# amoretti86/phylo

Measured on AMD Instinct MI355X. Metric: particle-site-likelihoods/sec, higher is better.
Workload: dtype f64; 1 GPU; primate.p N=12 S=898, GTR-init (jcmodel=false), K=2048 per GPU (K_total=2048), lambda=10, full sweep of 11 rank events; parallelism=particles sharded over 1 GPU(s), global resampling, sweeps_per_launch_set=16, contexts_in_flight=3, sweeps_in_flight=48, particles_in_flight=98304

## Files before the change

### phylo_amd/csrc/phylo_hip.hip

```cpp
#include "../../include/phylo_hip.h"

#include <cstring>
#include <hip/hip_runtime.h>
#include <hip/hip_ext.h>
#include <rocprim/device/device_radix_sort.hpp>

#include <cstdarg>
#include <cstdio>
#include <cstdlib>
#include <atomic>
#include <chrono>
#include <mutex>
#include <string>
#include <vector>

#include "phylo_comm.h"
#include "phylo_kernels.h"
#include "phylo_packed_codes.h"
#include "phylo_site_patterns.h"
#include "phylo_persist.h"
#include "phylo_grad.h"
#include "phylo_revlists_dev.h"
#include "phylo_sweep_plan.h"
#include "phylo_train.h"
// ... 27 lines not shown
    uint64_t seed = 0;
    uint32_t flags = 0;
    int M = 1, launches = 0, next_r = 0;
    bool active = false;
    int a_done_r = -1;
    sweep_plan plan{};
    sweep_chain_form chain{};
};

struct env_switches {
    bool eager_nodes = false, rehearse_sharded = false, replicated_book = false, no_leaf_codes = false, one_launch = false,
         persist_stamps = false, grad_one_stream = false, grad_two_streams = false, rev_host_lists = false, no_remote_cache = false,
         no_p2p = false, grad_rows_chain = false, grad_coeff_chain = false, tree_wide_keys = false;
    int persist_wgs = 0;
    unsigned long long p2p_wait_ticks = PK_P2P_WAIT_TICKS;
    size_t p2p_copy_words = 65536;
    int persist_nt = 256;
    int remote_cache_cap = 0;
    int scan_multi_min = 4096;
    int scan_ancestors = 1;
    int site_patterns = PK_PAT_AUTO;
    int clade_patterns = PK_CLADE_AUTO;
    int trees_chunk = 0;
    int launch_xcd = 0;
    int rell_chunk = 0;
    void read() {
        eager_nodes = getenv("PHYLO_EAGER_NODES") != nullptr;
        rehearse_sharded = getenv("PHYLO_REHEARSE_SHARDED") != nullptr;
        replicated_book = getenv("PHYLO_REPLICATED_BOOK") != nullptr;
        grad_rows_chain = getenv("PHYLO_GRAD_ROWS_CHAIN") != nullptr;
        grad_coeff_chain = getenv("PHYLO_GRAD_COEFF_CHAIN") != nullptr;
        no_leaf_codes = getenv("PHYLO_NO_LEAF_CODES") != nullptr;
        one_launch = getenv("PHYLO_ONE_LAUNCH") != nullptr;
        persist_stamps = getenv("PHYLO_PERSIST_STAMPS") != nullptr;
        grad_one_stream = getenv("PHYLO_GRAD_ONE_STREAM") != nullptr;
        grad_two_streams = getenv("PHYLO_GRAD_TWO_STREAMS") != nullptr;
        rev_host_lists = getenv("PHYLO_REV_HOST_LISTS") != nullptr;
        no_remote_cache = getenv("PHYLO_NO_REMOTE_CACHE") != nullptr;
        { const char* e = getenv("PHYLO_TREE_WIDE_KEYS"); tree_wide_keys = e && atoi(e) != 0; }
        { const char* e = getenv("PHYLO_REMOTE_CACHE_CAP"); remote_cache_cap = e ? atoi(e) : 0; }
        { const char* e = getenv("PHYLO_SITE_PATTERNS"); site_patterns = !e ? PK_PAT_AUTO : !strcmp(e, "force") ? PK_PAT_FORCE : atoi(e) == 0 ? PK_PAT_OFF : PK_PAT_AUTO; }
        { const char* e = getenv("PHYLO_CLADE_PATTERNS"); clade_patterns = !e ? PK_CLADE_AUTO : !strcmp(e, "force") ? PK_CLADE_FORCE : atoi(e) == 0 ? PK_CLADE_OFF : PK_CLADE_AUTO; }
        { const char* e = getenv("PHYLO_SCAN_MULTI_MIN"); scan_multi_min = e ? atoi(e) : 4096; }
        { const char* e = getenv("PHYLO_SCAN_ANCESTORS"); scan_ancestors = e ? atoi(e) : 1; }
        { const char* e = getenv("PHYLO_TREES_CHUNK"); trees_chunk = e ? atoi(e) : 0; }
        { const char* e = getenv("PHYLO_RELL_CHUNK"); rell_chunk = e ? atoi(e) : 0; }
        { const char* e = getenv("PHYLO_LAUNCH_XCD"); launch_xcd = !e ? 0 : atoi(e) > 0 ? atoi(e) : -1; }
        { const char* e = getenv("PHYLO_P2P"); no_p2p = e && atoi(e) == 0; }
        { const char* e = getenv("PHYLO_P2P_COPY_WORDS"); p2p_copy_words = e ? (size_t)atol(e) : 65536; }
        { const char* e = getenv("PHYLO_P2P_WAIT_S"); p2p_wait_ticks = e && atof(e) > 0 ? (unsigned long long)(atof(e) * 1e8) : PK_P2P_WAIT_TICKS; }
        const char* w = getenv("PHYLO_PERSIST_WGS");
        persist_wgs = w ? atoi(w) : 0;
        const char* t = getenv("PHYLO_PERSIST_NT");
        persist_nt = persist_nt_of(t ? atoi(t) : 0);
    }
};

struct phylo_ctx {
    int device = 0;
    env_switches env;
    int n_cus = 0;
    unsigned long long* d_rdraw = nullptr;
    unsigned long long* d_pctr = nullptr;
    unsigned long long pctr_base = 0;
    int pctr_Wg = 0, pctr_G = 0;
    bool pctr_dirty = false;
    int persist_blocks_per_cu = -1;
    bool last_persistent = false;
    int last_pp_nt = 0, last_pp_Wg = 0, last_pp_m = 0;
    size_t last_pp_lds = 0;
    unsigned long long* d_stamps = nullptr;
    int K = 0, N = 0, S = 0, A = 4;
    int Kloc = 0, k0 = 0;
    int rank = 0, world = 1;
    uint32_t flags = 0;
    hipStream_t stream = nullptr;
    hipEvent_t ev0 = nullptr, ev1 = nullptr;
    std::vector<hipEvent_t> kev;
    std::string err;
    bool have_leaves = false, have_model = false, swept = false, state_ready = false;
    int jc = 0;
    std::vector<double> h_lam_l, h_lam_r, h_ldf;
    double *d_Q = nullptr, *d_pi = nullptr, *d_lam_l = nullptr, *d_lam_r = nullptr, *d_ldf = nullptr;
    double* d_leaves = nullptr;
    uint8_t* d_leaf_codes = nullptr;
    uint8_t* d_leaf_packed = nullptr;
    uint8_t* d_pat = nullptr;
    int pat_U = 0;
    bool leaves_coded = false;
    uint8_t* d_clade = nullptr;
    uint8_t* h_clade_p = nullptr;
    size_t clade_cap = 0;
    pk_clade_layout clade_layout{};
    bool clade_ready = false;
    hipEvent_t ev_clade = nullptr;
    int32_t* d_bits[2] = {nullptr, nullptr};
    uint32_t* d_pair_hist = nullptr;
    bool hist_ready = false, codes_valid = false;
    double* d_pool = nullptr;
    double* d_nodell = nullptr;
    double *d_bl = nullptr, *d_br = nullptr, *d_Pmat = nullptr;
    double *d_logw = nullptr, *d_ll = nullptr;
    double* d_aux = nullptr;
    unsigned long long* d_rec = nullptr;
    int tile_override = 0;
    int site_tile = 0, ntiles = 1;
    double* d_tilev = nullptr;
    double* d_lse = nullptr;
    uint64_t* d_group_seeds = nullptr;
    char* d_tables = nullptr;
    int32_t *d_roots[2] = {nullptr, nullptr}, *d_cnt[2] = {nullptr, nullptr};
    double* d_rootll[2] = {nullptr, nullptr};
    const char** d_tab_ptrs = nullptr;
    int32_t* d_child = nullptr;
    unsigned int* d_mark = nullptr;
    double* d_sync = nullptr;
    bool p2p = false;
    char* d_xslab = nullptr;
    size_t xslab_bytes = 0, x_flag_off[2] = {0, 0};
    char** d_xslab_ptrs = nullptr;
    unsigned long long x_epoch[2] = {0, 0};
    bool last_lazy = false;
    bool leaves_newer = false;
    int32_t* d_merges = nullptr;
    int64_t* d_anc = nullptr;
    uint64_t* d_cdf[2] = {nullptr, nullptr};
    int32_t* d_anc_next = nullptr;
    int32_t* d_adopt_list = nullptr;
    int32_t* d_adopt_cnt = nullptr;
    int last_chain = 0;
    unsigned int* d_counter = nullptr;
    const double** d_pool_ptrs = nullptr;
    int32_t* d_mirror = nullptr;
    double* d_cache = nullptr;
    int cache_cap = 0;
    int32_t *d_roots_ad = nullptr, *d_cnt_ad = nullptr;
    double *d_rootll_ad = nullptr, *d_chosen = nullptr, *d_tw_b = nullptr, *d_tw_P = nullptr, *d_pot = nullptr;
    size_t tw_capacity = 0;
    double* d_twbuf = nullptr;
    size_t twbuf_cap = 0;
    double *d_htw_b = nullptr, *d_htw_P = nullptr, *d_hpot = nullptr, *d_hchosen = nullptr;
    int32_t* d_hroots_ad = nullptr;
    double *d_tau = nullptr, *d_ctw = nullptr, *d_twpart = nullptr, *d_twnode = nullptr;
    int64_t* d_joff = nullptr;
    size_t htw_rows = 0;
    std::vector<int64_t> h_joff;
    bool last_graph_twist = false, last_graph_marks = false;
    bool last_graph_eager = false;
    int last_M = 1;
    int32_t *d_hroots = nullptr, *d_hcnt = nullptr, *d_pos = nullptr;
    double* d_hrootll = nullptr;
    double *d_adj = nullptr, *d_om = nullptr, *d_G = nullptr, *d_C = nullptr, *d_part = nullptr, *d_nodeg = nullptr;
    double *d_leafpi = nullptr, *d_leafterm = nullptr, *d_terms = nullptr, *d_gout = nullptr;
    int32_t *d_ad_off = nullptr, *d_ad_idx = nullptr, *d_par_off = nullptr, *d_par_idx = nullptr;
    int32_t *d_heavy = nullptr, *d_chunk_beg = nullptr, *d_chunk_cnt = nullptr;
    int32_t *d_slow_flag = nullptr, *d_slow_idx = nullptr, *d_adp = nullptr;
    bool graph_ready = false, last_graph = false;
    int last_G = 1;
    bool last_final_missing = false;
    std::vector<uint64_t> h_group_seeds;
    int64_t* h_anc_p = nullptr;
    std::vector<int64_t> h_anc_glob;
    std::vector<double> h_gout;
    double* h_model_p = nullptr;
    double* h_leaves_p = nullptr;
    hipEvent_t ev_leaves = nullptr;
// ... 344 lines not shown
        HIPCHK(c, hipHostGetDevicePointer((void**)&c->hd_csr, c->h_csr_p, 0));
        HIPCHK(c, hipHostGetDevicePointer((void**)&c->hd_anc, c->h_anc_p, 0));
        HIPCHK(c, hipHostGetDevicePointer((void**)&c->hd_child, c->h_child_p, 0));
        HIPCHK(c, hipHostMalloc((void**)&c->h_pub, 16));
        HIPCHK(c, hipHostGetDevicePointer((void**)&c->hd_pub, c->h_pub, 0));
        HIPCHK(c, hipEventCreateWithFlags(&c->ev_gcopy, hipEventDisableTiming));
        HIPCHK(c, hipHostMalloc((void**)&c->h_dlmeta, ((size_t)PG_DL_META_INTS(R) + 4) * 4));
        c->h_dlmeta[PG_DL_META_INTS(R)] = 0;
        HIPCHK(c, hipHostGetDevicePointer((void**)&c->hd_dlmeta, c->h_dlmeta, 0));
        HIPCHK(c, hipEventCreateWithFlags(&c->ev_dl, hipEventDisableTiming));
        c->dl_temp_nn = 0;
        const pg_lists D = pg_lists_carve(c->d_ad_off, R, K);
        c->d_ad_idx = D.ad_idx; c->d_par_off = D.par_off; c->d_par_idx = D.par_idx;
        c->d_heavy = D.heavy; c->d_chunk_beg = D.chunk_beg; c->d_chunk_cnt = D.chunk_cnt;
        c->d_slow_flag = D.slow_flag; c->d_slow_idx = D.slow_idx; c->d_adp = D.adp;
    }
    if (c->world > 1) {
        const size_t Kl = c->Kloc, W = c->world;
        CHK(dalloc(c, &c->d_gchild, R * K * 2));
        CHK(dalloc(c, &c->d_gbl, R * K));
        CHK(dalloc(c, &c->d_gbr, R * K));
        CHK(dalloc(c, &c->d_gPmat, R * K * 32));
        CHK(dalloc(c, &c->d_ganc, (R > 1 ? R - 1 : 1) * K));
        c->gx_seg = R * Kl * 36 + (R > 1 ? (R - 1) * Kl : 0);
        c->gx_cl = c->gx_seg < PHYLO_SHM_SLOT / 8 ? c->gx_seg : PHYLO_SHM_SLOT / 8;
        const size_t words = (c->gx_seg + c->gx_cl - 1) / c->gx_cl * c->gx_cl * W;
        void* buf = nullptr;
        if (hipExtMallocWithFlags(&buf, words * 8, hipDeviceMallocFinegrained) != hipSuccess) {
            (void)hipGetLastError();
            HIPCHK(c, hipMalloc(&buf, words * 8));
        }
        c->d_gx = (unsigned long long*)buf;
        CHK(dalloc(c, &c->d_gx_src, W));
        std::vector<void*> src(W, buf);
        if (c->p2p) {
            int rc = phylo_comm_map_extra(c->comm, buf, &src, c->stream, &c->err);
            if (rc != PHYLO_OK) return rc;
        }
        HIPCHK(c, hipMemcpy((void*)c->d_gx_src, src.data(), W * sizeof(void*), hipMemcpyHostToDevice));
    }
    if (!c->evb0) {
        HIPCHK(c, hipEventCreate(&c->evb0));
        HIPCHK(c, hipEventCreate(&c->evb1));
        HIPCHK(c, hipStreamCreateWithFlags(&c->gstream, hipStreamNonBlocking));
        HIPCHK(c, hipEventCreateWithFlags(&c->ev_gfork, hipEventDisableTiming));
        HIPCHK(c, hipEventCreateWithFlags(&c->ev_gjoin, hipEventDisableTiming));
        HIPCHK(c, hipEventCreateWithFlags(&c->ev_gup, hipEventDisableTiming));
        {
            int least = 0, greatest = 0;
            HIPCHK(c, hipDeviceGetStreamPriorityRange(&least, &greatest));
            HIPCHK(c, hipStreamCreateWithPriority(&c->bgstream, hipStreamNonBlocking, least));
        }
        HIPCHK(c, hipEventCreateWithFlags(&c->ev_bgfork, hipEventDisableTiming));
        HIPCHK(c, hipEventCreateWithFlags(&c->ev_bgdone, hipEventDisableTiming));
        c->ev_coeff.assign((size_t)R, nullptr);
        for (auto& e : c->ev_coeff) HIPCHK(c, hipEventCreateWithFlags(&e, hipEventDisableTiming));
    }
    c->graph_ready = true;
    return PHYLO_OK;
}

template <typename... P, typename... A>
void launch_stamped(void (*kernel)(P...), dim3 grid, dim3 block, size_t lds, hipStream_t s, hipEvent_t e0, hipEvent_t e1, A&&... args) {
    if (e0) hipExtLaunchKernelGGL(kernel, grid, block, lds, s, e0, e1, 0, args...);
    else hipLaunchKernelGGL(kernel, grid, block, lds, s, args...);
}

static sweep_limits sweep_limits_of() {
    sweep_limits L{};
    L.max_groups = PK_MAX_GROUPS; L.twist_max_m = PK_TWIST_MAX_M; L.twist_max_j = PK_TWIST_MAX_J;
    L.mat_group = PK_MAT_GROUP; L.scan_fold_max_kg = PP_SCAN_KERNEL_MAX_KG; L.kept_bits_taxa = PG_KEPT_BITS_TAXA;
    L.scan_lds512_max_kg = 4096;
    L.one_tile_max_s = 4096;
    L.small_max_kg = 4096; L.small_max_kloc = 8192;
    L.book_packed8_min = 8192;
    L.sorted_min_draws = 262144;
    return L;
}
static const sweep_limits k_sweep_limits = sweep_limits_of();

int launch_scan(phylo_ctx* c, const double* logw, int Kg, int G, uint64_t* cdf, double* lse, int lse_stride, int logz_R = 0,
                const pp_anc_out* anc = nullptr) {
    const pp_anc_out ao = anc ? *anc : pp_anc_out{};
    const sweep_scan_form form = sweep_scan_form_of(Kg, c->env.scan_multi_min, cdf || lse, k_sweep_limits);
    if (ao.anc && (!cdf || logz_R > 0 || (form != SCAN_LDS_512 && form != SCAN_LDS_1024)))
        return fail(c, PHYLO_ESTATE, "launch_scan: the resampling outcome needs a cdf and a scan that holds it in LDS (Kg = %d)", Kg);
    if (form == SCAN_MULTI) {
        pp_scan_multi_args a{};
        a.logw = logw; a.Kg = Kg; a.B = (Kg + PP_SCAN_TILE - 1) / PP_SCAN_TILE;
        void* ws = nullptr;
        const size_t nb = (size_t)G * a.B;
        CHK(scratch_get(c, 11, (nb * 2 + (size_t)G * Kg) * 8, &ws));
        a.gmax = (double*)ws; a.bsum = (unsigned long long*)ws + nb; a.wbits = (unsigned long long*)ws + 2 * nb;
        a.cdf = (unsigned long long*)cdf; a.lse_out = lse; a.lse_stride = lse_stride; a.logz_R = logz_R;
        hipLaunchKernelGGL(pp_scan_multi_max, dim3(a.B, G), dim3(512), 0, c->stream, a);
        CHK(launch_check(c, "pp_scan_multi_max"));
        hipLaunchKernelGGL(pp_scan_multi_exp, dim3(a.B, G), dim3(512), 0, c->stream, a);
        CHK(launch_check(c, "pp_scan_multi_exp"));
        if (cdf) hipLaunchKernelGGL(pp_scan_multi_cdf, dim3(a.B + 1, G), dim3(512), 0, c->stream, a);
        else { a.lse_only = 1; hipLaunchKernelGGL(pp_scan_multi_cdf, dim3(1, G), dim3(512), 0, c->stream, a); }
        return launch_check(c, "pp_scan_multi_cdf");
    }
    if (form == SCAN_LDS_512) {
        if (ao.anc) hipLaunchKernelGGL(pp_resample_scan_anc<512>, dim3(G), dim3(512), pp_resample_scan_lds(Kg, true), c->stream, logw, Kg, cdf, lse, lse_stride, ao);
        else hipLaunchKernelGGL(pp_resample_scan<512>, dim3(G), dim3(512), pp_resample_scan_lds(Kg), c->stream, logw, Kg, cdf, lse, lse_stride, logz_R);
        return launch_check(c, "pp_resample_scan");
    }
    if (form == SCAN_LDS_1024) {
        const size_t lds = pp_resample_scan_lds(Kg, ao.anc != nullptr);
        static bool raised = false, raised_anc = false;
        if (lds > 65536 && !raised && !ao.anc) {
            HIPCHK(c, hipFuncSetAttribute((const void*)pp_resample_scan<1024>, hipFuncAttributeMaxDynamicSharedMemorySize,
                                          (int)pp_resample_scan_lds(PP_SCAN_KERNEL_MAX_KG)));
            raised = true;
        }
        if (ao.anc) {
            if (lds > 65536 && !raised_anc) {
                HIPCHK(c, hipFuncSetAttribute((const void*)pp_resample_scan_anc<1024>, hipFuncAttributeMaxDynamicSharedMemorySize,
                                              (int)pp_resample_scan_lds(PP_SCAN_KERNEL_MAX_KG, true)));
                raised_anc = true;
            }
            hipLaunchKernelGGL(pp_resample_scan_anc<1024>, dim3(G), dim3(1024), lds, c->stream, logw, Kg, cdf, lse, lse_stride, ao);
            return launch_check(c, "pp_resample_scan_anc");
        }
        hipLaunchKernelGGL(pp_resample_scan<1024>, dim3(G), dim3(1024), lds, c->stream, logw, Kg, cdf, lse, lse_stride, logz_R);
        return launch_check(c, "pp_resample_scan");
    }
    if (G > 1) hipLaunchKernelGGL(pk_resample_scan_groups, dim3(G), dim3(PK_COLS), 0, c->stream, logw, Kg, cdf, lse, lse_stride);
    else hipLaunchKernelGGL(pk_resample_scan, dim3(1), dim3(PK_COLS), 0, c->stream, logw, Kg, cdf, lse);
    return launch_check(c, "pk_resample_scan");
}

int wait_event_spin(phylo_ctx* c, hipEvent_t ev) {
    const auto t0 = std::chrono::steady_clock::now();
    for (;;) {
        const hipError_t e = hipEventQuery(ev);
        if (e == hipSuccess) return PHYLO_OK;
        if (e != hipErrorNotReady) return fail(c, PHYLO_EHIP, "hipEventQuery: %s", hipGetErrorString(e));
        if (std::chrono::steady_clock::now() - t0 > std::chrono::milliseconds(2)) break;
        __builtin_ia32_pause();
    }
    HIPCHK(c, hipEventSynchronize(ev));
    return PHYLO_OK;
}

int tile_for(const phylo_ctx* c, int S) { return c->tile_override ? c->tile_override : pm_site_tile(S); }

int refresh_leaf_ll(phylo_ctx* c) {
    if (!(c->have_leaves && c->have_model && c->state_ready)) return PHYLO_OK;
    hipLaunchKernelGGL(pk_row_loglik, dim3(c->N), dim3(64), 0, c->stream, c->d_leaves, c->d_pi, c->S, c->site_tile,
                       c->d_nodell);
    return launch_check(c, "pk_row_loglik(leaves)");
}

}

extern "C" {

const char* phylo_version(void) { return "phylo_hip 0.1 (gfx950)"; }

const char* phylo_last_error(const phylo_ctx* ctx) { return ctx ? ctx->err.c_str() : g_last_error.c_str(); }

int phylo_device_count(void) {
    int n = 0;
    if (hipGetDeviceCount(&n) != hipSuccess) return 0;
    return n;
}

int phylo_create(const int* device_ids, int n_gpus, int K, int N, int S, int A, uint32_t flags,
                 phylo_ctx** out) {
    if (!out) return fail(nullptr, PHYLO_EINVAL, "out is NULL");
    *out = nullptr;
    if (n_gpus != 1)
        return fail(nullptr, PHYLO_EINVAL, "n_gpus must be 1 (one process per GPU; join ranks with phylo_comm_init)");
    if (A != 4) return fail(nullptr, PHYLO_EINVAL, "A must be 4 (DNA alphabet), got %d", A);
    if (K < 1 || N < 2 || S < 1) return fail(nullptr, PHYLO_EINVAL, "need K >= 1, N >= 2, S >= 1 (K=%d N=%d S=%d)", K, N, S);
    if (N > PK_MAX_TAXA) return fail(nullptr, PHYLO_EINVAL, "N = %d exceeds the supported maximum %d", N, PK_MAX_TAXA);
    if ((double)(N - 1) * K + N > 2.0e9) return fail(nullptr, PHYLO_EINVAL, "node ids overflow int32");
    int ndev = 0;
    hipError_t e = hipGetDeviceCount(&ndev);
    if (e != hipSuccess || ndev < 1)
        return fail(nullptr, PHYLO_ENODEVICE, "no HIP device available (%s); this library has no CPU path",
                    e != hipSuccess ? hipGetErrorString(e) : "device count 0");
    const int dev = device_ids ? device_ids[0] : 0;
    if (dev < 0 || dev >= ndev) return fail(nullptr, PHYLO_ENODEVICE, "device id %d out of range [0,%d)", dev, ndev);
    phylo_ctx* c = new phylo_ctx();
    c->device = dev;
    c->K = K; c->N = N; c->S = S; c->A = A;
    c->Kloc = K; c->k0 = 0;
    c->flags = flags;
    c->env.read();
    {
        const char* t = getenv("PHYLO_SITE_TILE");
        int T = t ? atoi(t) : pm_site_tile(S);
        if (T < 64 || (T & 63) || T > PK_MAX_SITE_TILE) { delete c; return fail(nullptr, PHYLO_EINVAL, "PHYLO_SITE_TILE must be a multiple of 64 in [64, %d] (got %d)", PK_MAX_SITE_TILE, T); }
        c->tile_override = t ? T : 0;
        c->site_tile = T;
        c->ntiles = (S + T - 1) / T;
    }
    int rc = PHYLO_OK;
    do {
        if ((rc = bind(c)) != PHYLO_OK) break;
        {
            hipDeviceProp_t prop;
            if (hipGetDeviceProperties(&prop, dev) != hipSuccess) { rc = fail(c, PHYLO_EHIP, "hipGetDeviceProperties failed"); break; }
            c->n_cus = prop.multiProcessorCount;
        }
        if (hipStreamCreateWithFlags(&c->stream, hipStreamNonBlocking) != hipSuccess) { rc = fail(c, PHYLO_EHIP, "hipStreamCreate failed"); break; }
        if (hipEventCreate(&c->ev0) != hipSuccess || hipEventCreate(&c->ev1) != hipSuccess) { rc = fail(c, PHYLO_EHIP, "hipEventCreate failed"); break; }
        if ((rc = dalloc(c, &c->d_Q, 20 + 2 * (size_t)N)) != PHYLO_OK) break;
        c->d_pi = c->d_Q + 16;
        c->d_lam_l = c->d_Q + 20;
        c->d_lam_r = c->d_Q + 20 + N;
        if ((rc = dalloc(c, &c->d_ldf, (size_t)N + 1)) != PHYLO_OK) break;
        if ((rc = dalloc(c, &c->d_leaves, (size_t)N * S * 4)) != PHYLO_OK) break;
        if ((rc = dalloc(c, &c->d_leaf_codes, pk_leaf_image_bytes(N, S))) != PHYLO_OK) break;
        c->d_leaf_packed = c->d_leaf_codes + pk_packed_offset(N, S);
        c->d_pat = c->d_leaf_codes + pk_pat_offset(N, S);
        c->h_ldf.resize((size_t)N + 1);
        for (int cnt = 0; cnt <= N; ++cnt) c->h_ldf[cnt] = host_log_double_factorial(2 * (cnt > 2 ? cnt : 2) - 3);
        if (hipMemcpy(c->d_ldf, c->h_ldf.data(), ((size_t)N + 1) * 8, hipMemcpyHostToDevice) != hipSuccess) { rc = fail(c, PHYLO_EHIP, "ldf upload failed"); break; }
    } while (0);
    if (rc != PHYLO_OK) {
        g_last_error = c->err;
        phylo_destroy(c);
        return rc;
    }
    *out = c;
    return PHYLO_OK;
}

int phylo_destroy(phylo_ctx* c) {
    if (!c) return PHYLO_OK;
    (void)hipSetDevice(c->device);
    if (c->stream) (void)hipStreamSynchronize(c->stream);
    if (c->gstream) (void)hipStreamSynchronize(c->gstream);
    if (c->bgstream) (void)hipStreamSynchronize(c->bgstream);
    phylo_comm_destroy(&c->comm);
    free_sweep_state(c);
    void* ptrs[] = {c->d_Q, c->d_ldf, c->d_leaves, c->d_leaf_codes, c->d_clade};
    for (void* p : ptrs)
        if (p) (void)hipFree(p);
    for (auto& b : c->scratch)
        if (b.p) (void)hipFree(b.p);
    for (hipEvent_t e : c->kev) (void)hipEventDestroy(e);
    if (c->ev0) (void)hipEventDestroy(c->ev0);
    if (c->ev1) (void)hipEventDestroy(c->ev1);
    if (c->evb0) (void)hipEventDestroy(c->evb0);
    if (c->evb1) (void)hipEventDestroy(c->evb1);
    if (c->ev_model) (void)hipEventDestroy(c->ev_model);
    if (c->ev_tb0) (void)hipEventDestroy(c->ev_tb0);
    if (c->ev_tb1) (void)hipEventDestroy(c->ev_tb1);
    if (c->ev_tl0) (void)hipEventDestroy(c->ev_tl0);
    if (c->ev_tl1) (void)hipEventDestroy(c->ev_tl1);
    if (c->ev_rl0) (void)hipEventDestroy(c->ev_rl0);
    if (c->ev_rl1) (void)hipEventDestroy(c->ev_rl1);
    if (c->ev_rm0) (void)hipEventDestroy(c->ev_rm0);
    if (c->ev_rm1) (void)hipEventDestroy(c->ev_rm1);
    if (c->ev_tg0) (void)hipEventDestroy(c->ev_tg0);
    if (c->ev_tg1) (void)hipEventDestroy(c->ev_tg1);
    if (c->ev_tr0) (void)hipEventDestroy(c->ev_tr0);
    if (c->ev_tr1) (void)hipEventDestroy(c->ev_tr1);
    if (c->ev_tn0) (void)hipEventDestroy(c->ev_tn0);
    if (c->ev_tn1) (void)hipEventDestroy(c->ev_tn1);
    if (c->ev_tm0) (void)hipEventDestroy(c->ev_tm0);
    if (c->ev_tm1) (void)hipEventDestroy(c->ev_tm1);
    if (c->ev_tq0) (void)hipEventDestroy(c->ev_tq0);
    if (c->ev_tq1) (void)hipEventDestroy(c->ev_tq1);
    if (c->ev_ta0) (void)hipEventDestroy(c->ev_ta0);
    if (c->ev_ta1) (void)hipEventDestroy(c->ev_ta1);
    if (c->ev_ts0) (void)hipEventDestroy(c->ev_ts0);
    if (c->ev_ts1) (void)hipEventDestroy(c->ev_ts1);
    if (c->ev_gfork) (void)hipEventDestroy(c->ev_gfork);
    if (c->ev_gjoin) (void)hipEventDestroy(c->ev_gjoin);
    if (c->ev_gup) (void)hipEventDestroy(c->ev_gup);
    if (c->ev_bgfork) (void)hipEventDestroy(c->ev_bgfork);
    if (c->ev_bgdone) (void)hipEventDestroy(c->ev_bgdone);
    if (c->bgstream) (void)hipStreamDestroy(c->bgstream);
    for (hipEvent_t e : c->ev_coeff)
        if (e) (void)hipEventDestroy(e);
    if (c->gstream) (void)hipStreamDestroy(c->gstream);
    if (c->h_model_p) (void)hipHostFree(c->h_model_p);
    if (c->ev_leaves) (void)hipEventDestroy(c->ev_leaves);
    if (c->h_leaves_p) (void)hipHostFree(c->h_leaves_p);
    if (c->ev_clade) (void)hipEventDestroy(c->ev_clade);
    if (c->h_clade_p) (void)hipHostFree(c->h_clade_p);
    if (c->stream) (void)hipStreamDestroy(c->stream);
    delete c;
    return PHYLO_OK;
}

int phylo_site_tile(int S) { return pm_site_tile(S); }

int phylo_get_site_tile(const phylo_ctx* c) { return c ? c->site_tile : 0; }

int phylo_set_site_tile(phylo_ctx* c, int T) {
    CHK(bind(c));
    if (T < 0 || (T & 63) || T > PK_MAX_SITE_TILE)
        return fail(c, PHYLO_EINVAL, "the site tile must be a multiple of 64 in [64, %d], or 0 for the default (got %d)", PK_MAX_SITE_TILE, T);
    if (c->comm.transport != 0) return fail(c, PHYLO_ESTATE, "phylo_set_site_tile must precede phylo_comm_init (peers map the sweep state)");
    HIPCHK(c, hipStreamSynchronize(c->stream));
    c->tile_override = T;
    c->site_tile = T ? T : pm_site_tile(c->S);
    c->ntiles = (c->S + c->site_tile - 1) / c->site_tile;
// ... 1693 lines not shown
    const size_t lds = pp_layout(N, m, Kg).total;
    c->swept = false; ++c->sweep_serial;
    CHK(persist_chain(c, false));
    HIPCHK(c, hipEventRecord(c->ev0, c->stream));
    if (c->env.persist_nt == 512) hipLaunchKernelGGL((pp_sweep<512>), dim3(G * Wg), dim3(512), lds, c->stream, a);
    else hipLaunchKernelGGL((pp_sweep<256>), dim3(G * Wg), dim3(256), lds, c->stream, a);
    CHK(launch_check(c, "pp_sweep"));
    HIPCHK(c, hipEventRecord(c->ev1, c->stream));
    CHK(persist_chain(c, true));
    c->pctr_base += (unsigned long long)R * Wg;
    sweep_publish(c, true, false, G, false, 0, 1, (double)K * S * R);
    c->last_persistent = true;
    c->last_chain = 0;
    c->last_pp_nt = c->env.persist_nt; c->last_pp_Wg = Wg; c->last_pp_m = m; c->last_pp_lds = lds;
    return PHYLO_OK;
}


int phylo_sweep_begin(phylo_ctx* c, uint64_t seed, uint32_t flags, int M) { return sweep_begin_impl(c, seed, flags, M, nullptr, 1); }

static int comm_exchange(phylo_ctx* c, double* const* arrays, int n_arrays, size_t count, int purpose) {
    if (c->comm.transport == 0) return PHYLO_OK;
    if (!c->p2p) {
        if (n_arrays == 0) { double* rows[1] = {c->d_sync}; return phylo_comm_allgather_inplace(c->comm, rows, 1, 1, c->stream, &c->err); }
        return phylo_comm_allgather_inplace(c->comm, arrays, n_arrays, count, c->stream, &c->err);
    }
    if (n_arrays > 4) return fail(c, PHYLO_EINVAL, "comm_exchange: at most four arrays");
    pk_p2p_args a{};
    a.slabs = c->d_xslab_ptrs; a.world = c->world; a.me = c->rank;
    a.n_seg = n_arrays; a.seg_count = (int)count;
    for (int i = 0; i < n_arrays; ++i) {
        const ptrdiff_t off = (const char*)arrays[i] - c->d_xslab;
        if (off < 0 || (size_t)off + (size_t)c->world * count * 8 > c->xslab_bytes) return fail(c, PHYLO_EINVAL, "comm_exchange: array outside the exchange slab");
        a.seg_off[i] = (size_t)off;
    }
    a.flag_off = c->x_flag_off[purpose];
    a.epoch = ++c->x_epoch[purpose];
    a.timeout_word = c->d_counter + 1;
    a.wait_ticks = c->env.p2p_wait_ticks;
    const size_t words = (size_t)n_arrays * count * (size_t)(c->world - 1);
    if (words > c->env.p2p_copy_words) {
        const size_t wgs = (words + 4095) / 4096;
        hipLaunchKernelGGL(pk_p2p_copy, dim3((unsigned)(wgs < 512 ? wgs : 512)), dim3(1024), 0, c->stream, a);
        CHK(launch_check(c, "pk_p2p_copy"));
        a.n_seg = 0;
    }
    hipLaunchKernelGGL(pk_p2p_exchange, dim3(1), dim3(1024), 0, c->stream, a);
    return launch_check(c, "pk_p2p_exchange");
}

static bool pat_on(const phylo_ctx* c) { return pk_pat_take(c->S, c->pat_U, c->leaves_coded, c->ntiles, c->env.site_patterns); }

static pk_rank_args rank_args(const phylo_ctx* c, int r) {
    const sweep_plan& p = c->run.plan;
    const int N = c->N, K = c->K, Kl = c->Kloc, cur = r & 1, nxt = cur ^ 1;
    const size_t plane = (size_t)K * N;
    pk_rank_args b{};
    b.r = r; b.n = N - r; b.N = N; b.S = c->S; b.K = K; b.Kloc = Kl; b.k0 = c->k0;
    b.seed = c->run.seed; b.flags = c->run.flags;
    b.Kg = p.Kg; b.group_seeds = p.G > 1 ? c->d_group_seeds : nullptr;
    b.no_store = (r == p.R - 1 && p.no_store_last) ? 1 : 0;
    if (p.graph) {
        b.roots_old = c->d_hroots + plane * r; b.cnt_old = c->d_hcnt + plane * r;
        b.roots_new = c->d_hroots + plane * (r + 1); b.cnt_new = c->d_hcnt + plane * (r + 1);
        b.rootll_old = c->d_hrootll + plane * r; b.rootll_new = c->d_hrootll + plane * (r + 1);
        b.pos_hist = c->d_pos + plane * r;
    } else {
        b.roots_old = c->d_roots[cur]; b.cnt_old = c->d_cnt[cur];
        b.roots_new = c->d_roots[nxt]; b.cnt_new = c->d_cnt[nxt];
        b.rootll_old = c->d_rootll[cur]; b.rootll_new = c->d_rootll[nxt];
        if (p.clade_pat) { b.bits_old = c->d_bits[cur]; b.bits_new = c->d_bits[nxt]; }
    }
    if (p.local_book) {
        b.tab_ptrs = c->d_tab_ptrs;
        b.tab_off_rootll = (size_t)cur * K * N * 8;
        b.tab_off_roots = (size_t)16 * K * N + (size_t)cur * K * N * 4;
        b.tab_off_cnt = (size_t)24 * K * N + (size_t)cur * K * N * 4;
    }
    b.cdf = c->d_cdf[cur];
    b.rdraw = p.want_rdraw ? c->d_rdraw + (size_t)r * K : nullptr;
    b.ll_prev = r > 0 ? c->d_ll + (size_t)(r - 1) * K : nullptr;
    b.nodell = c->d_nodell;
    b.ldf = c->d_ldf; b.ldf_n = N;
    b.bl = c->d_bl; b.br = c->d_br;
    b.lam_l = c->h_lam_l[r]; b.lam_r = c->h_lam_r[r];
    b.loglam_l = pm_log(b.lam_l); b.loglam_r = pm_log(b.lam_r);
    b.ll_tilde0 = pm_log(1.0 / (double)p.Kg);
    b.leaves = c->d_leaves; b.pool = c->d_pool; b.pool_ptrs = c->d_pool_ptrs;
    b.mirror = (p.twist || p.replicated_book) ? nullptr : c->d_mirror; b.cache = c->d_cache; b.cache_cap = c->cache_cap;
    b.leaf_codes = c->leaves_coded ? c->d_leaf_codes : nullptr;
    b.leaf_packed = c->leaves_coded ? c->d_leaf_packed : nullptr;
    b.packed_leaf_bytes = pk_packed_leaf_bytes(c->S);
    b.Pmat = c->d_Pmat + (size_t)r * Kl * 32;
    b.pi = c->d_pi;
    b.logw_r = c->d_logw + (size_t)r * K;
    b.ll_r = c->d_ll + (size_t)r * K;
    b.merges = c->d_merges; b.ancestors = c->d_anc;
    b.child = c->d_child + (size_t)r * Kl * 2; b.aux = c->d_aux;
    b.rec = p.use_rec ? c->d_rec : nullptr;
    b.lazy = p.lazy ? 1 : 0; b.mark = c->d_mark; b.child_all = c->d_child; b.Pmat_all = c->d_Pmat;
    b.T = c->site_tile; b.ntiles = c->ntiles; b.tilev = c->d_tilev;
    if (c->run.chain.taken && r > 0) {
        b.anc_in = c->d_anc_next; b.adopt_list = c->d_adopt_list; b.adopt_cnt = c->d_adopt_cnt;
        b.item_waves = c->run.chain.item_waves; b.item_parts = c->run.chain.parts;
    }
    b.book_xcd = c->run.chain.taken && p.book_xcd;
    return b;
}

static int step_materialize(phylo_ctx* c, const pk_rank_args& b) {
    const sweep_plan& p = c->run.plan;
    const int Kl = c->Kloc, S = c->S;
    if (c->run.chain.taken) return PHYLO_OK;
    if (p.mat_by_draws) {
        const int grouped = p.mat_draws_grouped ? 1 : 0;
        hipLaunchKernelGGL(pk_materialize_by_draws, dim3(grouped ? Kl / PK_MAT_GROUP : Kl), dim3(PK_COLS), 0, c->stream, b, grouped);
        CHK(launch_check(c, "pk_materialize_by_draws"));
    } else {
        if (p.step_a_work) {
            hipLaunchKernelGGL(pk_all_marks, dim3(cdiv(c->K, 4)), dim3(64), 0, c->stream, b);
            CHK(launch_check(c, "pk_all_marks"));
        }
        if (p.mat_grouped) hipLaunchKernelGGL(pk_materialize_adopted_grouped, dim3(cdiv(Kl, PK_MAT_GROUP)), dim3(PK_COLS), 0, c->stream, b);
        else hipLaunchKernelGGL(pk_materialize_adopted, dim3(p.one_tile ? 1 : cdiv(S, PK_MAT_TILE), Kl), dim3(PK_COLS), 0, c->stream, b);
        CHK(launch_check(c, "pk_materialize_adopted"));
    }
    if (p.mat_barrier) CHK(comm_exchange(c, nullptr, 0, 0, 1));
    return PHYLO_OK;
}

static int sweep_step_a(phylo_ctx* c) {
    CHK(bind(c));
    if (!c->run.active) return fail(c, PHYLO_ESTATE, "phylo_sweep_step without phylo_sweep_begin");
    const int R = c->N - 1, r = c->run.next_r;
    if (r >= R) return fail(c, PHYLO_ESTATE, "all %d rank events of this sweep have been issued", R);
    c->run.a_done_r = r;
    if (!c->run.plan.step_a_work || r == 0) return PHYLO_OK;
    return step_materialize(c, rank_args(c, r));
}

static int step_twist(phylo_ctx* c, const pk_rank_args& b) {
    const sweep_plan& p = c->run.plan;
    const int N = c->N, K = c->K, Kl = c->Kloc, r = b.r;
    pk_twist_args ta{};
    ta.a = b;
    ta.M = c->run.M;
    ta.J = ((N - r) * (N - r - 1) / 2) * ta.M;
    ta.roots_ad = c->d_roots_ad; ta.cnt_ad = c->d_cnt_ad; ta.rootll_ad = c->d_rootll_ad;
    ta.tw_b = c->d_tw_b; ta.tw_P = c->d_tw_P; ta.pot = c->d_pot; ta.chosen = c->d_chosen;
    if (p.graph) {
        const size_t j0 = (size_t)c->h_joff[r];
        ta.tw_b = c->d_htw_b + j0 * 2; ta.tw_P = c->d_htw_P + j0 * 32; ta.pot = c->d_hpot + j0;
        ta.roots_ad = c->d_hroots_ad + (size_t)K * N * r; ta.chosen = c->d_hchosen + (size_t)r * K;
    }
    ta.Pmat_r = c->d_Pmat + (size_t)r * Kl * 32;
    ta.pair_hist = p.twist_ll ? c->d_pair_hist : nullptr;
    ta.codes = p.twist_ll ? c->d_leaf_codes : nullptr;
    ta.bl_r = c->d_bl + (size_t)r * Kl; ta.br_r = c->d_br + (size_t)r * Kl;
    ta.own_tables = p.twist_tables ? 0 : 1;
    ta.wbuf = c->d_twbuf;
    hipLaunchKernelGGL(pk_twist_adopt_draws, dim3(K + cdiv(2L * Kl * ta.J, 64)), dim3(64), 0, c->stream, ta, (const double*)c->d_Q, c->jc);
    CHK(launch_check(c, "pk_twist_adopt_draws"));
    if (p.twist_ll) {
        hipLaunchKernelGGL(pk_twist_potentials_ll, dim3((ta.J + 7) / 8, Kl), dim3(256), 0, c->stream, ta);
        CHK(launch_check(c, "pk_twist_potentials_ll"));
    }
// ... 59 lines not shown
        return launch_check(c, "pk_rank_book_chain");
    }
    const dim3 grid(cdiv(p.local_book ? c->Kloc : K, per));
    if (p.clade_pat) {
        if (w == 8) hipLaunchKernelGGL(pk_rank_book_packed_clade<8>, grid, dim3(64), lds * per, c->stream, b);
        else if (w == 16) hipLaunchKernelGGL(pk_rank_book_packed_clade<16>, grid, dim3(64), lds * per, c->stream, b);
        else return fail(c, PHYLO_ESTATE, "step_book: clade patterns at %d lanes", w);
        return launch_check(c, "pk_rank_book_packed");
    }
    switch (w) {
    case 8: hipLaunchKernelGGL(pk_rank_book_packed<8>, grid, dim3(64), lds * per, c->stream, b); break;
    case 16: hipLaunchKernelGGL(pk_rank_book_packed<16>, grid, dim3(64), lds * per, c->stream, b); break;
    case 32: hipLaunchKernelGGL(pk_rank_book_packed<32>, grid, dim3(64), lds * per, c->stream, b); break;
    case 64: hipLaunchKernelGGL(pk_rank_book_packed<64>, grid, dim3(64), lds * per, c->stream, b); break;
    default: return fail(c, PHYLO_ESTATE, "step_book: no pk_rank_book_packed of %d lanes", w);
    }
    return launch_check(c, "pk_rank_book_packed");
}

static int step_merge(phylo_ctx* c, const pk_rank_args& b) {
    const sweep_plan& p = c->run.plan;
    const int S = c->S;
    const dim3 mgrid((unsigned)((size_t)c->Kloc * c->ntiles));
    hipEvent_t e0 = nullptr, e1 = nullptr;
    if (p.timek && !p.twist) { e0 = c->kev[2 * b.r]; e1 = c->kev[2 * b.r + 1]; }
    if (!(b.lazy || b.no_store)) {
        const size_t lds = (size_t)(c->site_tile < S ? c->site_tile : S) * 8 + 16 + PK_STORE_STAGE_BYTES;
        launch_stamped(pk_rank_merge, mgrid, dim3(PK_COLS), lds, c->stream, e0, e1, b);
    } else if (b.rec) {
        pk_pi4 pi4;
        memcpy(pi4.v, c->h_model_p + 16, sizeof pi4.v);
        pk_pat_args pat = {nullptr, nullptr, 0, 0, 0u, 0u, nullptr};
        size_t lds = 0;
        if (p.clade_pat) {
            const pk_clade_layout& L = c->clade_layout;
            pat.clade = (const char*)c->d_clade + L.codes_bytes;
            pat.cstride = (unsigned int)L.stride; pat.crep = (unsigned int)L.rep_bytes;
            pat.rep_delta = (long long)(c->d_clade - c->d_leaf_packed);
            pat.U = c->pat_U;
            lds = pk_pat_lds_bytes(c->pat_U);
        } else if (pat_on(c)) {
            pat.pimg = (const char*)c->d_pat;
            pat.roff = (const char*)c->d_pat + pk_pat_image_bytes(S);
            pat.rep_delta = (long long)((c->d_pat + pk_pat_image_bytes(S) + pk_pat_rep_bytes()) - c->d_leaf_packed);
            pat.U = c->pat_U;
            lds = pk_pat_lds_bytes(c->pat_U);
        }
        const int n = (int)mgrid.x, grid = pk_launch_grid(n, 1, p.launch_xcd), n_xcd = p.launch_xcd ? -n : n;
        launch_stamped(pk_rank_merge_nostore, dim3((unsigned)grid), dim3(64), lds, c->stream, e0, e1, (const unsigned long long*)b.rec, b.Pmat,
                       S, b.T, b.ntiles, n_xcd, b.tilev, pi4, pat);
    } else {
        launch_stamped(pk_rank_merge_nostore_ids, mgrid, dim3(64), 0, c->stream, e0, e1, b);
    }
    return launch_check(c, "pk_rank_merge");
}

static int step_tiles(phylo_ctx* c, const pk_rank_args& b) {
    hipLaunchKernelGGL(pk_tile_epilogue, dim3(cdiv(c->Kloc, 256)), dim3(256), 0, c->stream, b);
    return launch_check(c, "pk_tile_epilogue");
}

static int step_exchange(phylo_ctx* c, int r) {
    const size_t K = c->K;
    double* rows[3] = {c->d_logw + r * K, c->d_ll + r * K, c->d_nodell + c->N + r * K};
    return comm_exchange(c, rows, 3, (size_t)c->Kloc, 0);
}

static int step_fix_rootll(phylo_ctx* c, int r) {
    const int N = c->N, K = c->K;
    double* rootll_new = c->run.plan.graph ? c->d_hrootll + (size_t)K * N * (r + 1) : c->d_rootll[(r & 1) ^ 1];
    hipLaunchKernelGGL(pk_fix_rootll, dim3(cdiv(K, 256)), dim3(256), 0, c->stream, rootll_new,
                       (const double*)(c->d_nodell + N + (size_t)r * K), K, N, N - r, c->k0, c->Kloc);
    return launch_check(c, "pk_fix_rootll");
}

static int step_scan(phylo_ctx* c, int r) {
    const sweep_plan& p = c->run.plan;
    const bool last = r + 1 == p.R;
    pp_anc_out ao{};
    if (c->run.chain.taken && !last) {
        ao.anc = c->d_anc_next; ao.list = c->d_adopt_list; ao.cnt = c->d_adopt_cnt;
        ao.group_seeds = p.G > 1 ? c->d_group_seeds : nullptr; ao.seed = c->run.seed; ao.r_next = (uint32_t)(r + 1);
    }
    return launch_scan(c, (const double*)(c->d_logw + (size_t)r * c->K), p.Kg, p.G, last ? (uint64_t*)nullptr : c->d_cdf[(r & 1) ^ 1],
                       c->d_lse + r, p.lse_stride, (last && p.fold_logz) ? p.R : 0, ao.anc ? &ao : nullptr);
}

static int sweep_step_impl(phylo_ctx* c, int phase) {
    CHK(bind(c));
    if (!c->run.active) return fail(c, PHYLO_ESTATE, "phylo_sweep_step without phylo_sweep_begin");
    const sweep_plan& p = c->run.plan;
    const int r = c->run.next_r;
    if (r >= p.R) return fail(c, PHYLO_ESTATE, "all %d rank events of this sweep have been issued", p.R);
    if (phase != 2) {
        if (c->run.a_done_r != r) CHK(sweep_step_a(c));
        const pk_rank_args b = rank_args(c, r);
        if (p.twist) CHK(step_twist(c, b));
        else CHK(step_book(c, b));
        if (p.mat_after_book && r > 0) CHK(step_materialize(c, b));
        CHK(step_merge(c, b));
        if (p.tile_epilogue) CHK(step_tiles(c, b));
    }
    if (phase == 0) CHK(step_exchange(c, r));
    if (phase == 1) return PHYLO_OK;
    if (p.fix_rootll) CHK(step_fix_rootll(c, r));
    CHK(step_scan(c, r));
    c->run.launches += sweep_plan_launches(p, r);
    ++c->run.next_r;
    return PHYLO_OK;
}

int phylo_sweep_step(phylo_ctx* c) { return sweep_step_impl(c, 0); }

int phylo_sweep_step_a(phylo_ctx* c) { return sweep_step_a(c); }

int phylo_sweep_step_group(phylo_ctx** ctxs, int n) {
    if (!ctxs || n < 1) return fail(nullptr, PHYLO_EINVAL, "phylo_sweep_step_group needs at least one context");
    for (int i = 0; i < n; ++i)
        if (!ctxs[i]) return fail(nullptr, PHYLO_EINVAL, "NULL context");
    if (n == 1 || ctxs[0]->comm.transport == 0) {
        for (int i = 0; i < n; ++i) CHK(sweep_step_impl(ctxs[i], 0));
        return PHYLO_OK;
    }
    for (int i = 0; i < n; ++i) {
        if (!ctxs[i]->run.active || ctxs[i]->run.next_r != ctxs[0]->run.next_r)
            return fail(ctxs[i], PHYLO_ESTATE, "the sweeps of a group must be at the same rank event");
        if (&phylo_comm_link(ctxs[i]->comm) != &phylo_comm_link(ctxs[0]->comm))
            return fail(ctxs[i], PHYLO_EINVAL, "the contexts of a group must share one communicator (phylo_comm_share)");
    }
    for (int i = 0; i < n; ++i) CHK(sweep_step_impl(ctxs[i], 1));
    std::vector<phylo_comm*> comms(n);
    std::vector<double*> rows((size_t)3 * n);
    std::vector<hipStream_t> streams(n);
    for (int i = 0; i < n; ++i) {
        phylo_ctx* c = ctxs[i];
        const size_t r = (size_t)c->run.next_r, K = c->K;
        comms[i] = &c->comm;
        streams[i] = c->stream;
        rows[3 * i] = c->d_logw + r * K;
        rows[3 * i + 1] = c->d_ll + r * K;
        rows[3 * i + 2] = c->d_nodell + c->N + r * K;
    }
    if (ctxs[0]->p2p) {
        for (int i = 0; i < n; ++i) {
            if (!ctxs[i]->p2p) return fail(ctxs[i], PHYLO_EINVAL, "the contexts of a group must use the same exchange");
            CHK(comm_exchange(ctxs[i], rows.data() + 3 * (size_t)i, 3, (size_t)ctxs[i]->Kloc, 0));
        }
    } else {
        phylo_ctx* c0 = ctxs[0];
        std::vector<size_t> counts(n);
        for (int i = 0; i < n; ++i) counts[i] = (size_t)ctxs[i]->Kloc;
        int rc = phylo_comm_allgather_group(comms.data(), rows.data(), 3, counts.data(), streams.data(), n, &c0->err);
        if (rc != PHYLO_OK) { g_last_error = c0->err; return rc; }
    }
    for (int i = 0; i < n; ++i) CHK(sweep_step_impl(ctxs[i], 2));
    return PHYLO_OK;
}

static int graph_gather(phylo_ctx* c) {
    const int K = c->K, Kl = c->Kloc, R = c->N - 1;
    pk_gx_args a{};
    a.world = c->world; a.me = c->rank; a.Kloc = Kl; a.K = K;
    a.seg = c->gx_seg; a.cl = c->gx_cl;
    a.xbuf = c->d_gx; a.xsrc = c->d_gx_src;
    int nf = 0;
    auto field = [&](const void* src, size_t stride, size_t off, void* dst, int rows, int w, int wide) {
        pk_gx_field& f = a.f[nf++];
// ... 970 lines not shown
    f.transport = transport != 0;
    sweep_facts_flags(f, flags);
    f.env_eager_nodes = switches & 1; f.env_rehearse_sharded = switches & 2; f.env_replicated_book = switches & 4;
    f.jc = switches & 8; f.coded_leaves = switches & 16; f.device_exchange = switches & 32; f.clade_tables = switches & 64;
    char why[160];
    if (sweep_refuses_batch(f, k_sweep_limits, why, sizeof why) || sweep_refuses_form(f, k_sweep_limits, why, sizeof why))
        return fail(nullptr, PHYLO_EINVAL, "%s", why);
    const sweep_plan p = sweep_plan_form(f, k_sweep_limits);
    *mask = sweep_plan_mask(p);
    for (int r = -1; r <= p.R; ++r) launches[r + 1] = sweep_plan_launches(p, r);
    return PHYLO_OK;
}

int phylo_debug_sweep_chain(int N, int K, int K_local, int S, int G, int M, int world, int transport, uint32_t flags, uint32_t switches,
                            int multi_min, int scan_ancestors, int32_t* out) {
    if (N < 2 || N > PK_MAX_TAXA || K < 1 || K_local < 1 || K_local > K || S < 1 || world < 1 || !out)
        return fail(nullptr, PHYLO_EINVAL, "phylo_debug_sweep_chain: bad arguments");
    sweep_facts f{};
    f.N = N; f.K = K; f.Kloc = K_local; f.S = S; f.G = G; f.M = M; f.world = world;
    f.ntiles = (S + pm_site_tile(S) - 1) / pm_site_tile(S);
    f.transport = transport != 0;
    sweep_facts_flags(f, flags);
    f.env_eager_nodes = switches & 1; f.env_rehearse_sharded = switches & 2; f.env_replicated_book = switches & 4;
    f.jc = switches & 8; f.coded_leaves = switches & 16; f.device_exchange = switches & 32;
    char why[160];
    if (sweep_refuses_batch(f, k_sweep_limits, why, sizeof why) || sweep_refuses_form(f, k_sweep_limits, why, sizeof why))
        return fail(nullptr, PHYLO_EINVAL, "%s", why);
    const sweep_chain_form ch = sweep_chain_form_of(sweep_plan_form(f, k_sweep_limits), S, multi_min, scan_ancestors, k_sweep_limits);
    out[0] = ch.taken ? 1 : 0; out[1] = ch.item_waves; out[2] = ch.parts;
    return PHYLO_OK;
}

int phylo_debug_sweep_launch(int N, int K, int K_local, int S, int G, int M, int world, int transport, uint32_t flags, uint32_t switches,
                             int launch_xcd, int32_t* out) {
    if (N < 2 || N > PK_MAX_TAXA || K < 1 || K_local < 1 || K_local > K || S < 1 || world < 1 || !out)
        return fail(nullptr, PHYLO_EINVAL, "phylo_debug_sweep_launch: bad arguments");
    sweep_facts f{};
    f.N = N; f.K = K; f.Kloc = K_local; f.S = S; f.G = G; f.M = M; f.world = world;
    f.ntiles = (S + pm_site_tile(S) - 1) / pm_site_tile(S);
    f.transport = transport != 0;
    sweep_facts_flags(f, flags);
    f.env_eager_nodes = switches & 1; f.env_rehearse_sharded = switches & 2; f.env_replicated_book = switches & 4;
    f.jc = switches & 8; f.coded_leaves = switches & 16; f.device_exchange = switches & 32; f.clade_tables = switches & 64;
    f.env_launch_xcd = launch_xcd;
    char why[160];
    if (sweep_refuses_batch(f, k_sweep_limits, why, sizeof why) || sweep_refuses_form(f, k_sweep_limits, why, sizeof why))
        return fail(nullptr, PHYLO_EINVAL, "%s", why);
    const sweep_plan p = sweep_plan_form(f, k_sweep_limits);
    out[0] = p.launch_xcd ? 1 : 0; out[1] = p.book_xcd ? 1 : 0;
    return PHYLO_OK;
}

int phylo_debug_sweep_launch_of(phylo_ctx* c, int32_t* out) {
    if (!c || !out) return fail(c, PHYLO_EINVAL, "phylo_debug_sweep_launch_of: NULL argument");
    const sweep_plan& p = c->run.plan;
    out[0] = p.launch_xcd ? 1 : 0; out[1] = p.book_xcd ? 1 : 0;
    return PHYLO_OK;
}

int phylo_debug_launch_map(int n, int W, int xcd, int32_t* grid, int32_t* items, int64_t cap) {
    if (n < 1 || (W != 1 && W != 2 && W != 4) || !grid)
        return fail(nullptr, PHYLO_EINVAL, "phylo_debug_launch_map: bad arguments");
    const int g = pk_launch_grid(n, W, xcd != 0);
    *grid = g;
    if (!items) return PHYLO_OK;
    if (cap < (int64_t)g * W) return fail(nullptr, PHYLO_EINVAL, "phylo_debug_launch_map: items needs %lld entries", (long long)g * W);
    for (int b = 0; b < g; ++b)
        for (int w = 0; w < W; ++w) items[(size_t)b * W + w] = pk_launch_item(b, g, W, w, xcd != 0);
    return PHYLO_OK;
}

int phylo_debug_sweep_chain_of(phylo_ctx* c, int32_t* taken) {
    if (!c || !taken) return fail(c, PHYLO_EINVAL, "phylo_debug_sweep_chain_of: NULL argument");
    *taken = c->last_chain;
    return PHYLO_OK;
}

int phylo_debug_scan_ancestors(phylo_ctx* c, const double* logw, int Kg, int G, const uint64_t* seeds, uint32_t r_next, int32_t* anc,
                               int32_t* list, int32_t* cnt) {
    CHK(bind(c));
    if (!logw || !seeds || !anc || !list || !cnt || Kg < 1 || G < 1 || G > PK_MAX_GROUPS)
        return fail(c, PHYLO_EINVAL, "phylo_debug_scan_ancestors: bad arguments");
    const size_t K = (size_t)Kg * G;
    void *dw, *dcdf, *dout, *dseed;
    CHK(scratch_get(c, 0, K * 8, &dw));
    CHK(scratch_get(c, 1, K * 8, &dcdf));
    CHK(scratch_get(c, 2, (2 * K + (size_t)G) * 4, &dout));
    CHK(scratch_get(c, 3, (size_t)G * 8, &dseed));
    HIPCHK(c, hipMemcpyAsync(dw, logw, K * 8, hipMemcpyHostToDevice, c->stream));
    HIPCHK(c, hipMemcpyAsync(dseed, seeds, (size_t)G * 8, hipMemcpyHostToDevice, c->stream));
    HIPCHK(c, hipMemsetAsync(dout, 0xff, (2 * K + (size_t)G) * 4, c->stream));
    pp_anc_out ao{};
    ao.anc = (int32_t*)dout; ao.list = ao.anc + K; ao.cnt = ao.list + K;
    ao.group_seeds = (const uint64_t*)dseed; ao.r_next = r_next;
    CHK(launch_scan(c, (const double*)dw, Kg, G, (uint64_t*)dcdf, (double*)nullptr, 0, 0, &ao));
    HIPCHK(c, hipMemcpyAsync(anc, ao.anc, K * 4, hipMemcpyDeviceToHost, c->stream));
    HIPCHK(c, hipMemcpyAsync(list, ao.list, K * 4, hipMemcpyDeviceToHost, c->stream));
    HIPCHK(c, hipMemcpyAsync(cnt, ao.cnt, (size_t)G * 4, hipMemcpyDeviceToHost, c->stream));
    HIPCHK(c, hipStreamSynchronize(c->stream));
    return PHYLO_OK;
}

int phylo_debug_pack_leaf_codes(const uint8_t* codes, int N, int S, uint8_t* packed, int64_t cap, int64_t* need) {
    if (N < 1 || S < 1 || !need || (packed && !codes)) return fail(nullptr, PHYLO_EINVAL, "phylo_debug_pack_leaf_codes: bad arguments");
    *need = (int64_t)pk_packed_bytes(N, S);
    if (!packed) return PHYLO_OK;
    if (cap < *need) return fail(nullptr, PHYLO_EINVAL, "phylo_debug_pack_leaf_codes: the image takes %lld bytes (got %lld)", (long long)*need, (long long)cap);
    pk_pack_leaf_codes(codes, N, S, packed);
    return PHYLO_OK;
}

int phylo_debug_site_patterns(const uint8_t* codes, int N, int S, int32_t* U, int32_t* rep, uint16_t* image, uint32_t* rep_off,
                              uint8_t* rep_leaf, int64_t rep_leaf_cap) {
    if (N < 1 || S < 1 || !codes || !U) return fail(nullptr, PHYLO_EINVAL, "phylo_debug_site_patterns: bad arguments");
    std::vector<int32_t> pat((size_t)S), rp((size_t)S);
    *U = pk_pat_columns(codes, N, S, pat.data(), rp.data());
    if (rep) memcpy(rep, rp.data(), (size_t)*U * sizeof(int32_t));
    if (image && *U <= PK_PAT_IMAGE_MAX_U) pk_pat_pack_image(pat.data(), S, *U, image);
    if (rep_off && *U <= PK_PAT_MAX_U) pk_pat_rep_offsets(rp.data(), *U, rep_off);
    if (rep_leaf && *U <= PK_PAT_MAX_U) {
        if (rep_leaf_cap < (int64_t)pk_packed_bytes(N, *U))
            return fail(nullptr, PHYLO_EINVAL, "phylo_debug_site_patterns: the representative leaf image takes %lld bytes (got %lld)",
                        (long long)pk_packed_bytes(N, *U), (long long)rep_leaf_cap);
        pk_pat_rep_leaf_image(codes, N, S, rp.data(), *U, rep_leaf, pk_packed_leaf_bytes(*U));
    }
    return PHYLO_OK;
}

int phylo_debug_site_patterns_rule(int S, int U, int coded, int ntiles, int sw) {
    if (S < 1 || U < 0 || ntiles < 1 || sw < PK_PAT_OFF || sw > PK_PAT_FORCE) {
        (void)fail(nullptr, PHYLO_EINVAL, "phylo_debug_site_patterns_rule: bad arguments");
        return -1;
    }
    return pk_pat_take(S, U, coded != 0, ntiles, sw) ? 1 : 0;
}

int phylo_debug_site_patterns_of(phylo_ctx* c, int32_t* U, int32_t* taken) {
    if (!c || !U || !taken) return fail(c, PHYLO_EINVAL, "phylo_debug_site_patterns_of: NULL argument");
    if (!c->have_leaves) return fail(c, PHYLO_ESTATE, "phylo_debug_site_patterns_of needs leaves");
    *U = c->pat_U;
    *taken = pat_on(c) ? 1 : 0;
    return PHYLO_OK;
}

int phylo_debug_clade_patterns_rule(int pat_taken, int N, int S, int U, int sw, int64_t* bytes) {
    if (N < 1 || S < 1 || U < 0 || sw < PK_CLADE_OFF || sw > PK_CLADE_FORCE) {
        (void)fail(nullptr, PHYLO_EINVAL, "phylo_debug_clade_patterns_rule: bad arguments");
        return -1;
    }
    if (bytes) *bytes = (int64_t)pk_clade_layout_of(N, S, U).total;
    return pk_clade_take(pat_taken != 0, N, S, U, sw) ? 1 : 0;
}

int phylo_debug_clade_tables(const uint8_t* codes, int N, int S, int32_t* U, int64_t* layout, uint8_t* tables, int64_t cap, uint16_t* cls) {
    if (N < 1 || N > PK_CLADE_MAX_N || S < 1 || !codes || !U || !layout) return fail(nullptr, PHYLO_EINVAL, "phylo_debug_clade_tables: bad arguments");
    std::vector<int32_t> pat((size_t)S), rp((size_t)S);
    *U = pk_pat_columns(codes, N, S, pat.data(), rp.data());
    const pk_clade_layout L = pk_clade_layout_of(N, S, *U);
    layout[0] = (int64_t)L.codes_bytes; layout[1] = (int64_t)L.rep_bytes; layout[2] = (int64_t)L.image_bytes;
    layout[3] = (int64_t)L.stride; layout[4] = (int64_t)L.total;
    if (!tables) return PHYLO_OK;
    if (*U > PK_PAT_MAX_U) return fail(nullptr, PHYLO_EINVAL, "phylo_debug_clade_tables: U = %d exceeds %d", *U, PK_PAT_MAX_U);
    if (cap < (int64_t)L.total) return fail(nullptr, PHYLO_EINVAL, "phylo_debug_clade_tables: the tables take %lld bytes (got %lld)", (long long)L.total, (long long)cap);
    pk_clade_build(codes, N, S, pat.data(), rp.data(), *U, tables, cls);
    return PHYLO_OK;
}

int phylo_debug_clade_patterns_of(phylo_ctx* c, int32_t* eligible, int32_t* taken, int64_t* bytes) {
    if (!c || !eligible || !taken || !bytes) return fail(c, PHYLO_EINVAL, "phylo_debug_clade_patterns_of: NULL argument");
    if (!c->have_leaves) return fail(c, PHYLO_ESTATE, "phylo_debug_clade_patterns_of needs leaves");
    *eligible = (c->clade_ready && pat_on(c)) ? 1 : 0;
    *taken = c->run.plan.clade_pat ? 1 : 0;
    *bytes = c->clade_ready ? (int64_t)c->clade_layout.total : 0;
    return PHYLO_OK;
}

int phylo_debug_tree_plan(int N, int K, int G, int world, int64_t n_clades, int64_t n_topologies, int kept_whole, int force_wide,
                          int64_t summary_temp, int64_t branches_temp, int64_t* scalars, int64_t* summary_slab, int64_t* branches_slab,
// ... 690 lines not shown
```

### phylo_amd/csrc/phylo_kernels.h

```cpp
#pragma once
#include <hip/hip_runtime.h>
#include <stdint.h>

#include "phylo_math.h"
#include "phylo_packed_codes.h"
#include "phylo_site_patterns.h"
#include "phylo_launch_map.h"

#define PK_COLS 256
#define PK_AUX 8
#define PK_MAX_TAXA 512
#define PK_MAX_GROUPS 64

enum { AUX_SUM_REM = 0, AUX_FPRIOR, AUX_LPRIOR, AUX_RPRIOR, AUX_LL_TILDE, AUX_PAREN, AUX_LOGV, AUX_Q };
#define PK_REC 16
enum { REC_BASE_L = PK_AUX, REC_BASE_R, REC_NODELL, REC_ROOTLL, REC_LL, REC_LOGW, REC_FLAGS  };
#define PK_REC_SLOTS (REC_FLAGS + 1)
static_assert(PK_REC_SLOTS <= PK_REC && PK_REC_SLOTS <= 16, "one lane per slot: with 16 lanes or more per particle the bookkeeping writes the record in one trip (pk_book_tail)");

__device__ __forceinline__ double pk_block_canon_sum(double col, double* sh4) {
#pragma unroll
    for (int off = 1; off < 64; off <<= 1) col = col + __shfl_xor(col, off, 64);
    __syncthreads();
    if ((threadIdx.x & 63) == 0) sh4[threadIdx.x >> 6] = col;
// ... 444 lines not shown
        if (lo + 8 <= K) {
            ulonglong2* q = reinterpret_cast<ulonglong2*>(cdf + lo);
            q[0] = make_ulonglong2(run + e[0], run + e[1]);
            q[1] = make_ulonglong2(run + e[2], run + e[3]);
            q[2] = make_ulonglong2(run + e[4], run + e[5]);
            q[3] = make_ulonglong2(run + e[6], run + e[7]);
        } else {
#pragma unroll
            for (int j = 0; j < 8; ++j)
                if (lo + j < K) cdf[lo + j] = run + e[j];
        }
        carry += ((sh->u4[0] + sh->u4[1]) + sh->u4[2]) + sh->u4[3];
    }
}

__global__ __launch_bounds__(PK_COLS) void pk_resample_scan(const double* logw, int K, uint64_t* __restrict__ cdf,
                                                             double* __restrict__ lse_out) {
    __shared__ pk_scan_lds sh;
    pk_scan_block(logw, K, cdf, lse_out, &sh);
}
__global__ __launch_bounds__(PK_COLS) void pk_resample_scan_groups(const double* logw, int K, uint64_t* __restrict__ cdf,
                                                                    double* __restrict__ lse_out, int lse_stride) {
    __shared__ pk_scan_lds sh;
    const int g = blockIdx.x;
    uint64_t* cg = cdf ? cdf + (size_t)g * K : nullptr;
    pk_scan_block(logw + (size_t)g * K, K, cg, lse_out + (size_t)g * lse_stride, &sh);
}

__device__ __forceinline__ int pk_cdf_search(const uint64_t* __restrict__ cdf, int K, uint64_t thr) {
    int lo = 0, hi = K;
    while (lo < hi) {
        const int mid = (lo + hi) >> 1;
        if (cdf[mid] > thr) hi = mid; else lo = mid + 1;
    }
    return lo < K ? lo : K - 1;
}

__global__ void pk_resample_search(const uint64_t* __restrict__ cdf, int K, int n_draw, int k0, uint64_t seed,
                                   uint32_t step, int64_t* __restrict__ idx) {
    const int k = blockIdx.x * blockDim.x + threadIdx.x;
    if (k >= n_draw) return;
    const pm_u32x4 x = pm_philox4x32((uint32_t)(k0 + k), step, PM_STREAM_RESAMPLE, 0u, seed);
    const uint64_t R = ((uint64_t)x.y << 32) | x.x;
    idx[k] = pk_cdf_search(cdf, K, pm_mulhi64(R, cdf[K - 1]));
}

__global__ void pk_logz_total(const double* __restrict__ lse, int R, double* __restrict__ out) {
    if (threadIdx.x == 0 && blockIdx.x == 0) {
        double z = 0.0;
        for (int r = 0; r < R; ++r) z = z + lse[r];
        *out = z;
    }
}

__global__ void pk_logz_total_groups(double* __restrict__ lse, int R, int stride) {
    if (threadIdx.x == 0) {
        double* l = lse + (size_t)blockIdx.x * stride;
        double z = 0.0;
        for (int r = 0; r < R; ++r) z = z + l[r];
        l[R] = z;
    }
}

__global__ void pk_init_tables(int32_t* __restrict__ roots, int32_t* __restrict__ cnt, double* __restrict__ rootll,
                               const double* __restrict__ nodell, int K, int N) {
    const int i = blockIdx.x * blockDim.x + threadIdx.x;
    if (i >= K * N) return;
    roots[i] = i % N;
    cnt[i] = 1;
    rootll[i] = nodell[i % N];
}

struct pk_rank_args {
    int r, n, N, S, K , Kloc, k0;
    uint64_t seed;
    uint32_t flags;
    const int32_t* roots_old; const int32_t* cnt_old;
    int32_t* roots_new; int32_t* cnt_new;
    const double* rootll_old; double* rootll_new;
    const uint64_t* cdf;
    const double* ll_prev;
    double* nodell;
    const double* ldf; int ldf_n;
    const double* bl; const double* br;
    double lam_l, lam_r, loglam_l, loglam_r, ll_tilde0;
    const double* leaves;
    const uint8_t* leaf_codes;
    const uint8_t* leaf_packed;
    size_t packed_leaf_bytes;
    double* pool;
    const double* const* pool_ptrs;
    int32_t* mirror;
    double* cache;
    int cache_cap;
    const double* Pmat;
    const double* pi;
    double* logw_r; double* ll_r;
    int32_t* merges;
    int64_t* ancestors;
    int lazy;
    unsigned int* mark;
    const int32_t* child_all;
    const double* Pmat_all;
    int32_t* child;
    double* aux;
    int32_t* pos_hist;
    const char* const* tab_ptrs;
    size_t tab_off_rootll, tab_off_roots, tab_off_cnt;
    int Kg;
    const uint64_t* group_seeds;
    int no_store;
    const unsigned long long* rdraw;
    int T, ntiles;
    double* tilev;
    unsigned long long* rec;
    const int32_t* anc_in;
    const int32_t* adopt_list;
    const int32_t* adopt_cnt;
    int item_waves, item_parts;
    int book_xcd;
    const int32_t* bits_old; int32_t* bits_new;
};

struct pk_book_lds {
    double *ord_ll, *ord_ldf, *hbl, *hbr, *anc_ll, *ldf;
    uint32_t* key; int32_t *ro, *co, *ord_cnt;
    double* aux; int32_t* misc;
    int32_t* bo;
};
__host__ __device__ inline size_t pk_book_lds_bytes(int N) {
    const size_t n4 = ((size_t)N + 3) & ~(size_t)3;
    return (6 * n4 + 4) * 8 + PK_AUX * 8 + (4 * n4) * 4 + 16 ;
}
__device__ __forceinline__ pk_book_lds pk_book_carve(char* base, int N) {
    const size_t n4 = ((size_t)N + 3) & ~(size_t)3;
    pk_book_lds L;
    L.ord_ll = (double*)base;
    L.ord_ldf = L.ord_ll + n4;
    L.hbl = L.ord_ldf + n4;
    L.hbr = L.hbl + n4;
    L.anc_ll = L.hbr + n4;
    L.ldf = L.anc_ll + n4;
    L.aux = L.ldf + n4 + 4;
    L.key = (uint32_t*)(L.aux + PK_AUX);
    L.ro = (int32_t*)(L.key + n4);
    L.co = L.ro + n4;
    L.ord_cnt = L.co + n4;
    L.misc = L.ord_cnt + n4;
    L.bo = nullptr;
    return L;
}
__host__ __device__ inline size_t pk_book_bits_lds_bytes(int N) { return (((size_t)N + 3) & ~(size_t)3) * 4; }
__device__ __forceinline__ pk_book_lds pk_book_carve_sub(char* smem, int sub, int groups, int N) {
    pk_book_lds L = pk_book_carve(smem + (size_t)sub * pk_book_lds_bytes(N), N);
    L.bo = (int32_t*)(smem + (size_t)groups * pk_book_lds_bytes(N) + (size_t)sub * pk_book_bits_lds_bytes(N));
    return L;
}

template <bool BITS = false>
__device__ __forceinline__ void pk_rec_write(const pk_rank_args& a, int k, int kg, int t, const pk_book_lds& L) {
    const size_t node_sz = (size_t)a.S * 4;
    unsigned long long v;
    if (t < PK_AUX) {
        v = (unsigned long long)__double_as_longlong(L.aux[t]);
    } else if (t <= REC_BASE_R) {
        const int id = L.misc[t - REC_BASE_L];
        if (id >= a.N) v = (unsigned long long)(a.pool + (size_t)(id - a.N) * node_sz);
        else if (a.leaf_codes) v = (unsigned long long)(a.leaf_packed + (size_t)id * a.packed_leaf_bytes);
        else v = (unsigned long long)(a.leaves + (size_t)id * node_sz);
    } else if (t == REC_NODELL) {
        v = (unsigned long long)(a.nodell + (a.N + a.r * a.K + kg));
    } else if (t == REC_ROOTLL) {
        v = (unsigned long long)(a.rootll_new + ((size_t)kg * a.N + (a.n - 2)));
    } else if (t == REC_LL) {
        v = (unsigned long long)(a.ll_r + kg);
    } else if (t == REC_LOGW) {
        v = (unsigned long long)(a.logw_r + kg);
    } else {
        v = a.leaf_codes ? (unsigned long long)((L.misc[0] < a.N ? 1 : 0) | (L.misc[1] < a.N ? 2 : 0)) : 0ull;
        if constexpr (BITS) v |= (unsigned long long)(unsigned int)L.misc[2] << 2;
    }
    a.rec[(size_t)k * PK_REC + t] = v;
}


template <int LP>
__device__ __forceinline__ int pk_cdf_search_group(const uint64_t* cdf, int K, uint64_t R, int sl, int lane) {
    const int gshift = lane & ~(LP - 1);
    const unsigned long long gmask = LP == 64 ? ~0ull : ((1ull << (LP & 63)) - 1ull);
    int lo = 0, hi = K;
    int step = (K + LP - 1) / LP;
    int p = (sl + 1) * step - 1;
    if (p > K - 1) p = K - 1;
    const uint64_t total = cdf[K - 1];
    uint64_t c = cdf[p];
    const uint64_t thr = pm_mulhi64(R, total);
    bool done = false;
    for (;;) {
        const unsigned long long ball = __ballot(!done && c > thr);
        if (!done) {
            const unsigned long long mask = (ball >> gshift) & gmask;
            const int f = mask ? __ffsll((long long)mask) - 1 : LP - 1;
            int pf = lo + (f + 1) * step - 1;
            if (pf > hi - 1) pf = hi - 1;
            lo = lo + f * step;
            hi = pf + 1;
            if (lo >= hi) lo = hi - 1;
            if (hi - lo <= 1) done = true;
            else {
                step = (hi - lo + LP - 1) / LP;
                p = lo + (sl + 1) * step - 1;
                if (p > hi - 1) p = hi - 1;
                c = cdf[p];
            }
        }
        if (__all(done)) break;
    }
    return lo;
}

template <int LP, bool KEY_LOOP, bool ANC_IN = false, bool BITS = false>
__device__ __forceinline__ void pk_book_packed(const pk_rank_args& a, int kg, bool local, const pk_book_lds& L, int sl, int lane) {
    const int n = a.n, N = a.N, k = kg - a.k0;
    const int grp = a.group_seeds ? kg / a.Kg : 0;
    const int gbase = grp * a.Kg;
    const uint64_t seed = a.group_seeds ? a.group_seeds[grp] : a.seed;
    const uint32_t kin = (uint32_t)(kg - gbase);
    {
        #pragma unroll 1
        for (int j = sl; j <= a.r; j += LP) {
            L.hbl[j] = local ? a.bl[(size_t)j * a.Kloc + k] : 0.0;
            L.hbr[j] = local ? a.br[(size_t)j * a.Kloc + k] : 0.0;
        }
        #pragma unroll 1
        for (int j = sl; j <= a.ldf_n; j += LP) L.ldf[j] = a.ldf[j];
        const int nb = (n + 3) / 4;
        uint64_t Rdraw;
        if (ANC_IN) Rdraw = 0;
        if (KEY_LOOP && nb > LP - 1) {
            #pragma unroll 1
            for (int b = sl; b < nb; b += LP) {
                const pm_u32x4 x = pm_philox4x32(kin, (uint32_t)a.r, PM_STREAM_PAIR, (uint32_t)b, seed);
                L.key[b * 4 + 0] = x.x; L.key[b * 4 + 1] = x.y; L.key[b * 4 + 2] = x.z; L.key[b * 4 + 3] = x.w;
            }
            if (!ANC_IN) {
                const pm_u32x4 x = pm_philox4x32(kin, (uint32_t)a.r, PM_STREAM_RESAMPLE, 0u, seed);
                Rdraw = ((uint64_t)x.y << 32) | x.x;
            }
        } else {
            const bool res = !ANC_IN && sl == LP - 1;
            const pm_u32x4 x = pm_philox4x32(kin, (uint32_t)a.r, res ? PM_STREAM_RESAMPLE : PM_STREAM_PAIR, res ? 0u : (uint32_t)sl, seed);
            if (sl < nb) { L.key[sl * 4 + 0] = x.x; L.key[sl * 4 + 1] = x.y; L.key[sl * 4 + 2] = x.z; L.key[sl * 4 + 3] = x.w; }
            if (!ANC_IN) {
                const int src = (lane & ~(LP - 1)) + LP - 1;
                Rdraw = ((uint64_t)(uint32_t)__shfl((int)x.y, src, 64) << 32) | (uint32_t)__shfl((int)x.x, src, 64);
            }
        }
        int anc = kg;
        if (ANC_IN) { if (a.r > 0) anc = gbase + a.anc_in[kg]; }
        else if (a.r > 0) anc = gbase + pk_cdf_search_group<LP>(a.cdf + gbase, a.group_seeds ? a.Kg : a.K, Rdraw, sl, lane);
        const int32_t* ro = a.roots_old + (size_t)anc * N;
        const int32_t* co = a.cnt_old + (size_t)anc * N;
        const double* rl = a.rootll_old + (size_t)anc * N;
        if (a.tab_ptrs) {
            const char* base = a.tab_ptrs[anc / a.Kloc];
            ro = reinterpret_cast<const int32_t*>(base + a.tab_off_roots) + (size_t)anc * N;
            co = reinterpret_cast<const int32_t*>(base + a.tab_off_cnt) + (size_t)anc * N;
            rl = reinterpret_cast<const double*>(base + a.tab_off_rootll) + (size_t)anc * N;
        }
        #pragma unroll 1
        for (int i = sl; i < n; i += LP) { L.ro[i] = ro[i]; L.co[i] = co[i]; L.anc_ll[i] = rl[i]; }
        if constexpr (BITS) {
            const int32_t* bo = a.bits_old + (size_t)anc * N;
            #pragma unroll 1
            for (int i = sl; i < n; i += LP) L.bo[i] = bo[i];
        }
        if (sl == 0) {
            L.misc[3] = anc;
            if (local) L.aux[AUX_LL_TILDE] = (a.r > 0) ? a.ll_prev[anc] : a.ll_tilde0;
        }
    }
    __syncthreads();
    {
        unsigned long long best = 0ull;
        #pragma unroll 1
        for (int i = sl; i < n; i += LP) {
            const unsigned long long c = ((unsigned long long)L.key[i] << 32) | (0xffffffffu - (uint32_t)i);
            best = c > best ? c : best;
        }
#pragma unroll
        for (int off = 1; off < LP; off <<= 1) {
            const unsigned long long o = __shfl_xor(best, off, 64);
            best = o > best ? o : best;
        }
        const int il = (int)(0xffffffffu - (uint32_t)best);
        best = 0ull;
        #pragma unroll 1
        for (int i = sl; i < n; i += LP) {
            const unsigned long long c = ((unsigned long long)L.key[i] << 32) | (0xffffffffu - (uint32_t)i);
            if (i != il) best = c > best ? c : best;
        }
#pragma unroll
        for (int off = 1; off < LP; off <<= 1) {
            const unsigned long long o = __shfl_xor(best, off, 64);
            best = o > best ? o : best;
        }
        const int ir = (int)(0xffffffffu - (uint32_t)best);
        int32_t* rn = a.roots_new + (size_t)kg * N;
        int32_t* cn = a.cnt_new + (size_t)kg * N;
        double* rln = a.rootll_new + (size_t)kg * N;
        #pragma unroll 1
        for (int i = sl; i < n; i += LP) {
            if (i == il || i == ir) continue;
            const unsigned long long mine = ((unsigned long long)L.key[i] << 32) | (uint32_t)i;
            int rank = 0;
            #pragma unroll 1
            for (int j = 0; j < n; ++j) {
                const unsigned long long cj = ((unsigned long long)L.key[j] << 32) | (uint32_t)j;
                rank += (j != il && j != ir && cj < mine) ? 1 : 0;
            }
            const int node = L.ro[i], c = L.co[i];
            const double xll = L.anc_ll[i];
            rn[rank] = node;
            cn[rank] = c;
            rln[rank] = xll;
            if (a.pos_hist) a.pos_hist[(size_t)kg * N + i] = rank;
            L.ord_cnt[rank] = c;
            L.ord_ll[rank] = xll;
            L.ord_ldf[rank] = L.ldf[c < a.ldf_n ? c : a.ldf_n];
            if constexpr (BITS) a.bits_new[(size_t)kg * N + rank] = L.bo[i];
        }
        if (sl == 0) {
            if constexpr (BITS) {
                const int bnew = L.bo[il] | L.bo[ir];
                a.bits_new[(size_t)kg * N + (n - 2)] = bnew;
                L.misc[2] = bnew;
            }
            const int cnew = L.co[il] + L.co[ir];
            rn[n - 2] = N + a.r * a.K + kg;
            cn[n - 2] = cnew;
            L.ord_cnt[n - 2] = cnew;
            L.ord_ldf[n - 2] = L.ldf[cnew < a.ldf_n ? cnew : a.ldf_n];
            L.misc[0] = L.ro[il];
            L.misc[1] = L.ro[ir];
            if (a.pos_hist) { a.pos_hist[(size_t)kg * N + il] = -1; a.pos_hist[(size_t)kg * N + ir] = -1; }
            if (local) {
                a.merges[((size_t)a.r * a.Kloc + k) * 2 + 0] = il;
                a.merges[((size_t)a.r * a.Kloc + k) * 2 + 1] = ir;
                if (a.r > 0) a.ancestors[(size_t)(a.r - 1) * a.Kloc + k] = L.misc[3] - gbase;
            }
        }
    }
    __syncthreads();
    if (local) {
        const double* src = sl == 0 ? L.ord_ll : sl == 1 ? L.ord_ldf : sl == 2 ? L.hbl : L.hbr;
        const int cnt = sl == 0 ? n - 2 : sl == 1 ? n - 1 : sl < 4 ? a.r + 1 : 0;
        const double ca = sl == 0 ? 1.0 : sl == 1 ? -1.0 : sl == 2 ? -a.lam_l : -a.lam_r;
        const double cb = sl == 2 ? a.loglam_l : sl == 3 ? a.loglam_r : 0.0;
        const int trips = n - 1 > a.r + 1 ? n - 1 : a.r + 1;
        double acc = 0.0;
        #pragma unroll 1
        for (int j = 0; j < trips; ++j)
            if (j < cnt) acc = acc + (ca * src[j] + cb);
        int vminus = 0;
        #pragma unroll 1
        for (int p = sl; p < n - 1; p += LP) {
            const int c = L.ord_cnt[p];
            vminus += c - (c == 1 ? 1 : 0);
        }
#pragma unroll
        for (int off = 1; off < LP; off <<= 1) vminus += __shfl_xor(vminus, off, 64);
        const double q = 1.0 / ((double)((n - 1) * n) / 2.0);
        const double lg = pm_log(sl == 0 ? (double)vminus : q);
        if (sl == 0) {
            const double b_l = L.hbl[a.r], b_r = L.hbr[a.r];
            L.aux[AUX_SUM_REM] = acc;
            L.aux[AUX_PAREN] = ((a.loglam_l - a.lam_l * b_l) + a.loglam_r) - a.lam_r * b_r;
            L.aux[AUX_LOGV] = lg;
        } else if (sl == 1) {
            L.aux[AUX_FPRIOR] = acc;
            L.aux[AUX_Q] = (a.flags & 1u) ? q : lg;
        } else if (sl == 2) {
            L.aux[AUX_LPRIOR] = acc;
        } else if (sl == 3) {
            L.aux[AUX_RPRIOR] = acc;
        }
    }
    __syncthreads();
}

__device__ __forceinline__ bool pk_remote_node(const pk_rank_args& a, int id, int& x, const double*& src) {
    if (id < a.N) return false;
    x = id - a.N;
    const int rho = x / a.K, kap = x - rho * a.K, owner = kap / a.Kloc;
    if (owner * a.Kloc == a.k0) return false;
    src = a.pool_ptrs[owner] + ((size_t)rho * a.Kloc + (kap - owner * a.Kloc)) * (size_t)a.S * 4;
    return true;
}
__device__ __forceinline__ int pk_cache_claim(const pk_rank_args& a, int id) {
    int x;
    const double* src;
    if (!pk_remote_node(a, id, x, src)) return -1;
    if (__hip_atomic_load(a.mirror + x, __ATOMIC_RELAXED, __HIP_MEMORY_SCOPE_AGENT) != 0) return -1;
    int expected = 0;
    if (!__hip_atomic_compare_exchange_strong(a.mirror + x, &expected, -1, __ATOMIC_RELAXED, __ATOMIC_RELAXED, __HIP_MEMORY_SCOPE_AGENT)) return -1;
    const int slot = __hip_atomic_fetch_add(a.mirror + (size_t)(a.N - 1) * a.K, 1, __ATOMIC_RELAXED, __HIP_MEMORY_SCOPE_AGENT);
    if (slot >= a.cache_cap) {
        __hip_atomic_store(a.mirror + x, -2, __ATOMIC_RELAXED, __HIP_MEMORY_SCOPE_AGENT);
        return -1;
    }
    return slot;
}
__device__ __forceinline__ void pk_cache_fill(const pk_rank_args& a, int id, int slot, int lane) {
    typedef __attribute__((ext_vector_type(4))) unsigned int cu4;
    typedef __attribute__((address_space(1))) const cu4 gsrc_t;
    typedef __attribute__((address_space(1))) cu4 gdst_t;
    int x;
    const double* srcd;
    pk_remote_node(a, id, x, srcd);
    const char* src = (const char*)srcd;
    char* dst = (char*)(a.cache + (size_t)slot * (size_t)a.S * 4);
    const size_t bytes = (size_t)a.S * 32;
    size_t o = (size_t)lane * 16;
    for (; o + 3 * 1024 < bytes; o += 4 * 1024) {
        const cu4 v0 = *(gsrc_t*)(src + o), v1 = *(gsrc_t*)(src + o + 1024), v2 = *(gsrc_t*)(src + o + 2048), v3 = *(gsrc_t*)(src + o + 3072);
        *(gdst_t*)(dst + o) = v0; *(gdst_t*)(dst + o + 1024) = v1; *(gdst_t*)(dst + o + 2048) = v2; *(gdst_t*)(dst + o + 3072) = v3;
    }
    for (; o < bytes; o += 1024) *(gdst_t*)(dst + o) = *(gsrc_t*)(src + o);
    if (lane == 0) __hip_atomic_store(a.mirror + x, slot + 1, __ATOMIC_RELAXED, __HIP_MEMORY_SCOPE_AGENT);
}

template <int LP, bool BITS = false>
__device__ __forceinline__ void pk_book_tail(const pk_rank_args& a, int kg, bool local, bool mark, bool cache, const pk_book_lds& L,
                                             int sl, int lane) {
    if (local) {
        const int k = kg - a.k0;
#pragma unroll
        for (int t = sl; t < PK_AUX + 2; t += LP) {
            if (t < PK_AUX) a.aux[(size_t)k * PK_AUX + t] = L.aux[t];
            else a.child[k * 2 + (t - PK_AUX)] = L.misc[t - PK_AUX];
        }
        if (a.rec) {
#pragma unroll
            for (int t = sl; t < PK_REC_SLOTS; t += LP) pk_rec_write<BITS>(a, k, kg, t, L);
        }
    }
    if (mark && sl == 0) a.mark[(size_t)(a.r - 1) * a.K + L.misc[3]] = 1u;
    if (cache) {
#pragma unroll
        for (int c = 0; c < 2; ++c) {
            const int id = L.misc[c];
            const int slot = (local && sl == 0) ? pk_cache_claim(a, id) : -1;
            for (int g2 = 0; g2 < 64 / LP; ++g2) {
                const int s2 = __shfl(slot, g2 * LP, 64), id2 = __shfl(id, g2 * LP, 64);
                if (s2 >= 0) pk_cache_fill(a, id2, s2, lane);
            }
// ... 640 lines not shown
            pm_lp_mul2(col, xa, xb);
        } else {
            pm_lp_mul(col, xa);
        }
    }
}

__global__ __launch_bounds__(64) __attribute__((amdgpu_waves_per_eu(7, 8))) void pk_rank_merge_nostore_ids(const pk_rank_args a) {
    __shared__ __attribute__((aligned(16))) double tabL[5][4], tabR[5][4];
    __shared__ double lik25[25];
    const int item = (int)blockIdx.x, ntiles = a.ntiles;
    const int k = ntiles == 1 ? item : item / ntiles, tau = item - k * ntiles;
    const int s0 = tau * a.T, s1 = s0 + a.T < a.S ? s0 + a.T : a.S;
    const double* Pu = a.Pmat + (size_t)k * 32;
    PK_TOUCH_DECL;
    PK_TOUCH_256_2(Pu, a.pi, a.aux + (size_t)k * PK_AUX);
    int cl = a.child[k * 2];
    const int cr = a.child[k * 2 + 1];
    PK_TOUCH_END(cl);
    const bool codedL = a.leaf_codes && cl < a.N, codedR = a.leaf_codes && cr < a.N;
    const double* Lp = pk_node_ptr(a, cl);
    const double* Rp = pk_node_ptr(a, cr);
    const uint8_t* Lc = a.leaf_codes + (codedL ? (size_t)cl * a.S : 0);
    const uint8_t* Rc = a.leaf_codes + (codedR ? (size_t)cr * a.S : 0);
    double Pl[16], Pr[16];
#pragma unroll
    for (int u = 0; u < 16; ++u) { Pl[u] = Pu[u]; Pr[u] = Pu[16 + u]; }
    const double pi[4] = {a.pi[0], a.pi[1], a.pi[2], a.pi[3]};
    pm_lp col = pm_lp_init();
    if (codedL) {
        if (codedR) pk_rows_loop<true, true>(s0, s1, Lp, Rp, Lc, Rc, Pu, a.pi, Pl, Pr, tabL, tabR, lik25, pi, col);
        else pk_rows_loop<true, false>(s0, s1, Lp, Rp, Lc, Rc, Pu, a.pi, Pl, Pr, tabL, tabR, lik25, pi, col);
    } else {
        if (codedR) pk_rows_loop<false, true>(s0, s1, Lp, Rp, Lc, Rc, Pu, a.pi, Pl, Pr, tabL, tabR, lik25, pi, col);
        else pk_rows_loop<false, false>(s0, s1, Lp, Rp, Lc, Rc, Pu, a.pi, Pl, Pr, tabL, tabR, lik25, pi, col);
    }
    const double tot = pk_wave_tree_sum(pm_lp_finish(col));
    if (threadIdx.x == 0) {
        typedef __attribute__((address_space(4))) const pk_rank_args pk_kernarg;
        pk_kernarg* ka = (pk_kernarg*)__builtin_amdgcn_kernarg_segment_ptr();
        if (ka->ntiles != 1) {
            ka->tilev[(size_t)k * ka->ntiles + tau] = tot;
        } else {
            const int kg = ka->k0 + k;
            const double* ax = ka->aux + (size_t)k * PK_AUX;
            const double fl = ax[AUX_SUM_REM] + tot;
            const double ll = ((fl + ax[AUX_FPRIOR]) + ax[AUX_LPRIOR]) + ax[AUX_RPRIOR];
            const double lw = (((ll - ax[AUX_LL_TILDE]) - ax[AUX_PAREN]) + ax[AUX_LOGV]) - ax[AUX_Q];
            const int N = ka->N, r = ka->r, K = ka->K;
            ka->nodell[N + r * K + kg] = tot;
            ka->rootll_new[(size_t)kg * N + (ka->n - 2)] = tot;
            ka->ll_r[kg] = ll;
            ka->logw_r[kg] = lw;
        }
    }
}

struct pk_pi4 { double v[4]; };
typedef __attribute__((address_space(1))) const double pk_gdc;
typedef __attribute__((address_space(1))) double pk_gd;
typedef __attribute__((address_space(4))) const unsigned long long pk_cu64;
typedef __attribute__((address_space(4))) const double pk_cdbl;
__device__ __forceinline__ void pk_leaf_vec(const double* __restrict__ P , int c, double (&t)[4]) {
    pk_load4(P + (c < 4 ? c : 0) * 4, t);
    if (c == 4) {
        double v[3][4];
#pragma unroll
        for (int i = 0; i < 3; ++i) pk_load4(P + (i + 1) * 4, v[i]);
#pragma unroll
        for (int j = 0; j < 4; ++j) t[j] = pm_fma(1.0, v[2][j], pm_fma(1.0, v[1][j], pm_fma(1.0, v[0][j], 1.0 * t[j])));
    }
}
__device__ __forceinline__ bool pk_build_lik25_direct(const double* __restrict__ Pu , const double (&pi)[4], double* lik25, int t) {
    bool special = false;
    if (t < 25) {
        const int cl = t / 5, cr = t - cl * 5;
        double tl[4], tr[4], o[4];
        pk_leaf_vec(Pu, cl, tl);
        pk_leaf_vec(Pu + 16, cr, tr);
#pragma unroll
        for (int j = 0; j < 4; ++j) o[j] = tl[j] * tr[j];
        const double x = pk_site_lik(pi, o);
        lik25[t] = x;
        special = pm_lp_special(x);
    }
    return special;
}
__device__ __forceinline__ unsigned int pk_cw_byte(const unsigned int (&w)[4], int j) { return (w[j >> 2] >> (8 * (j & 3))) & 0xffu; }
__device__ __forceinline__ bool pk_rows_fast_cc(int s0, int s1, const char* bl, const char* br, pk_cstream& c, const double* lik25,
                                                pm_lp& col) {
    const char* lb = (const char*)lik25;
    pm_lp_flag flag = pm_lp_flag_init();
    int n = __builtin_amdgcn_readfirstlane((s1 - s0 + 63) >> 6), Jc = __builtin_amdgcn_readfirstlane(s0 >> 10);
    #pragma unroll 1
    for (;;) {
        const unsigned int w[4] = {(c.nl.x * 5u + c.nr.x) * 8u, (c.nl.y * 5u + c.nr.y) * 8u, (c.nl.z * 5u + c.nr.z) * 8u,
                                   (c.nl.w * 5u + c.nr.w) * 8u};
        if (n > 16) pk_cs_request<true, true>(c, bl, br, Jc + 1);
#pragma unroll
        for (int j = 0; j < 16; j += 2) {
            if (n < j + 2) {
                if (n == j + 1) pm_lp_mul_normal(col, *(const double*)(lb + pk_cw_byte(w, j)));
                break;
            }
            const double xa = *(const double*)(lb + pk_cw_byte(w, j));
            const double xb = *(const double*)(lb + pk_cw_byte(w, j + 1));
            pm_lp_mul2_spec_q(col, xa, xb, flag);
        }
        if (n <= 16) break;
        n -= 16; ++Jc;
    }
    return pm_lp_flag_set(flag);
}
template <bool CL, bool CR>
__device__ __forceinline__ void pk_rows_pair_spec(pk_rowregs& A, pk_rowregs& B, unsigned int ca, unsigned int cb, int s, int s1,
                                                  const char* bl, const char* br, const double (&Pl)[16], const double (&Pr)[16],
                                                  const double (*tabL)[4], const double (*tabR)[4], const double (&pi)[4], pm_lp& col,
                                                  pm_lp_flag& flag) {
    pk_rows_load_u<CL, CR>(B, bl, br, s + 64, s1);
    (CL ? A.cl : A.cr) = ca;
    double xa = pk_rows_lik<CL, CR>(A, Pl, Pr, tabL, tabR, nullptr, pi);
    xa = s < s1 ? xa : 1.0;
    pk_rows_load_u<CL, CR>(A, bl, br, s + 128, s1);
    (CL ? B.cl : B.cr) = cb;
    double xb = pk_rows_lik<CL, CR>(B, Pl, Pr, tabL, tabR, nullptr, pi);
    xb = s + 64 < s1 ? xb : 1.0;
    pm_lp_mul2_spec(col, xa, xb, flag);
}
template <bool CL, bool CR>
__device__ __forceinline__ bool pk_rows_fast_mixed(int s0, int s1, const char* bl, const char* br, pk_rowregs& A, pk_cstream& c,
                                                   const double (&Pl)[16], const double (&Pr)[16], const double (*tabL)[4],
                                                   const double (*tabR)[4], const double (&pi)[4], pm_lp& col) {
    static_assert(CL != CR, "one coded side");
    pk_rowregs B;
    pm_lp_flag flag = pm_lp_flag_init();
    int s = s0 + (int)(threadIdx.x & 63);
    int n = __builtin_amdgcn_readfirstlane((s1 - s0 + 63) >> 6), Jc = __builtin_amdgcn_readfirstlane(s0 >> 10);
    #pragma unroll 1
    for (;;) {
        const pk_u4 q = CL ? c.nl : c.nr;
        unsigned long long lo = (unsigned long long)q.x | ((unsigned long long)q.y << 32);
        unsigned long long hi = (unsigned long long)q.z | ((unsigned long long)q.w << 32);
        if (n > 16) pk_cs_request<CL, CR>(c, bl, br, Jc + 1);
        const int m = n < 16 ? n : 16;
        #pragma unroll 1
        for (int t = 0; t < (m >> 1); ++t, s += 128) {
            if (t == 4) lo = hi;
            const unsigned int cw = (unsigned int)lo;
            pk_rows_pair_spec<CL, CR>(A, B, cw & 0xffu, (cw >> 8) & 0xffu, s, s1, bl, br, Pl, Pr, tabL, tabR, pi, col, flag);
            lo >>= 16;
        }
        if (m & 1) {
            if ((m >> 1) == 4) lo = hi;
            (CL ? A.cl : A.cr) = (unsigned int)lo & 0xffu;
            double xa = pk_rows_lik<CL, CR>(A, Pl, Pr, tabL, tabR, nullptr, pi);
            xa = s < s1 ? xa : 1.0;
            pm_lp_mul_spec(col, xa, flag);
        }
        if (n <= 16) break;
        n -= 16; ++Jc;
    }
    return pm_lp_flag_set(flag);
}
typedef __attribute__((address_space(1))) const unsigned int pk_gu32c;
template <bool CL, bool CR>
__device__ __forceinline__ void pk_pat_rows(pk_rowregs& x, const char* bl, const char* br, unsigned int off) {
    if constexpr (!CL) { x.l0 = *(pk_gu4c*)(bl + off); x.l1 = *(pk_gu4c*)(bl + off + 16u); }
    if constexpr (!CR) { x.r0 = *(pk_gu4c*)(br + off); x.r1 = *(pk_gu4c*)(br + off + 16u); }
}
template <bool CL, bool CR>
__device__ __forceinline__ void pk_pat_entry(pk_rowregs& X, unsigned int code, unsigned int u, unsigned int U, const double (&Pl)[16],
                                             const double (&Pr)[16], const double (*tabL)[4], const double (*tabR)[4],
                                             const double (&pi)[4], double* ulik, pm_lp_flag& flag) {
    if constexpr (CL) X.cl = code;
    if constexpr (CR) X.cr = code;
    double x = pk_rows_lik<CL, CR>(X, Pl, Pr, tabL, tabR, nullptr, pi);
    x = u < U ? x : 1.0;
    flag.f = pm_min_u32(flag.f, pm_lp_key(x));
    ulik[u] = x;
}
template <bool CL, bool CR>
__device__ __forceinline__ void pk_pat_phase1(int U, const char* bl, const char* br, const char* rl, const char* roff,
                                              const double (&Pl)[16], const double (&Pr)[16], const double (*tabL)[4],
                                              const double (*tabR)[4], const double (&pi)[4], double* ulik, pm_lp_flag& flag) {
    static_assert(!(CL && CR), "an uncoded side");
    const int nU = __builtin_amdgcn_readfirstlane((U + 63) >> 6);
    unsigned int u = threadIdx.x & 63u;
    unsigned long long lo = 0;
    if constexpr (CL || CR) {
        const pk_u4 q = *(pk_gu4c*)(rl + u * 16u);
        lo = (unsigned long long)q.x | ((unsigned long long)q.y << 32);
    }
    pk_rowregs A, B;
    unsigned int ro = *(pk_gu32c*)(roff + u * 4u);
    pk_pat_rows<CL, CR>(A, bl, br, ro);
    ro = *(pk_gu32c*)(roff + (u + 64u) * 4u);
    #pragma unroll 1
    for (int t = 0; t < (nU >> 1); ++t, u += 128u) {
        pk_pat_rows<CL, CR>(B, bl, br, ro);
        ro = *(pk_gu32c*)(roff + (u + 128u) * 4u);
        const unsigned int cw = (unsigned int)lo;
        pk_pat_entry<CL, CR>(A, cw & 0xffu, u, (unsigned int)U, Pl, Pr, tabL, tabR, pi, ulik, flag);
        pk_pat_rows<CL, CR>(A, bl, br, ro);
        ro = *(pk_gu32c*)(roff + (u + 192u) * 4u);
        pk_pat_entry<CL, CR>(B, (cw >> 8) & 0xffu, u + 64u, (unsigned int)U, Pl, Pr, tabL, tabR, pi, ulik, flag);
        lo >>= 16;
    }
    if (nU & 1) pk_pat_entry<CL, CR>(A, (unsigned int)lo & 0xffu, u, (unsigned int)U, Pl, Pr, tabL, tabR, pi, ulik, flag);
    if (threadIdx.x == 0) ulik[U] = 1.0;
}
__device__ __forceinline__ void pk_pat_request(pk_u4& n0, pk_u4& n1, const char* pimg, int Jc) {
    const unsigned int o = (unsigned int)Jc * (2u * PK_PAT_HALF_BYTES) + (threadIdx.x & 63u) * 16u;
    n0 = *(pk_gu4c*)(pimg + o);
    n1 = *(pk_gu4c*)(pimg + o + (unsigned int)PK_PAT_HALF_BYTES);
}
__device__ __forceinline__ void pk_pat_walk(int s1, const char* pimg, pk_u4 n0, pk_u4 n1, const double* ulik, pm_lp& col, pm_lp_flag& flag) {
    const char* ub = (const char*)ulik;
    int n = __builtin_amdgcn_readfirstlane((s1 + 63) >> 6), Jc = 0;
    #pragma unroll 1
    for (;;) {
        const unsigned int w[8] = {n0.x, n0.y, n0.z, n0.w, n1.x, n1.y, n1.z, n1.w};
        if (n > 16) pk_pat_request(n0, n1, pimg, Jc + 1);
#pragma unroll
        for (int j = 0; j < 16; j += 2) {
            if (n < j + 2) {
                if (n == j + 1) pm_lp_mul_normal(col, *(const double*)(ub + (w[j >> 1] & 0xffffu)));
                break;
            }
            const double xa = *(const double*)(ub + (w[j >> 1] & 0xffffu));
            const double xb = *(const double*)(ub + (w[j >> 1] >> 16));
            pm_lp_mul2_spec_q(col, xa, xb, flag);
        }
        if (n <= 16) break;
        n -= 16; ++Jc;
    }
}
struct pk_pat_args {
    const char* pimg; const char* roff; long long rep_delta ; int U;
    unsigned int cstride, crep;
    const char* clade;
};
typedef __attribute__((address_space(4))) const pk_pat_args pk_pat_kargs;
template <bool CL, bool CR>
__device__ __forceinline__ void pk_clade_rows(pk_rowregs& x, const char* bl, const char* br, const char* cb, unsigned int off) {
    pk_pat_rows<CL, CR>(x, bl, br, off);
    if constexpr (CL) x.cl = *(pk_gu8c*)(cb + (off >> 5));
    if constexpr (CR) x.cr = *(pk_gu8c*)(cb + (off >> 5));
}
template <bool CL, bool CR>
__device__ __forceinline__ void pk_clade_entry(const pk_rowregs& X, unsigned int u, unsigned int U, const double (&Pl)[16],
                                               const double (&Pr)[16], const double (*tabL)[4], const double (*tabR)[4],
                                               const double (&pi)[4], double* ulik, pm_lp_flag& flag) {
    double x = pk_rows_lik<CL, CR>(X, Pl, Pr, tabL, tabR, nullptr, pi);
    x = u < U ? x : 1.0;
    flag.f = pm_min_u32(flag.f, pm_lp_key(x));
    ulik[u] = x;
}
template <bool CL, bool CR>
__device__ __forceinline__ void pk_clade_phase1(const char* blk, const char* bl, const char* br, const char* cb, const double (&Pl)[16],
                                                const double (&Pr)[16], const double (*tabL)[4], const double (*tabR)[4],
                                                const double (&pi)[4], double* ulik, pm_lp_flag& flag) {
    static_assert(!(CL && CR), "an uncoded side");
    const char* roff = blk + PK_CLADE_HDR_BYTES;
    unsigned int u = threadIdx.x & 63u;
    pk_rowregs A, B;
    unsigned int ro = *(pk_gu32c*)(roff + u * 4u);
    const int U = *(__attribute__((address_space(4))) const int*)blk;
    pk_clade_rows<CL, CR>(A, bl, br, cb, ro);
    ro = *(pk_gu32c*)(roff + (u + 64u) * 4u);
    const int nU = (U + 63) >> 6;
    #pragma unroll 1
    for (int t = 0; t < (nU >> 1); ++t, u += 128u) {
        pk_clade_rows<CL, CR>(B, bl, br, cb, ro);
        ro = *(pk_gu32c*)(roff + (u + 128u) * 4u);
        pk_clade_entry<CL, CR>(A, u, (unsigned int)U, Pl, Pr, tabL, tabR, pi, ulik, flag);
        pk_clade_rows<CL, CR>(A, bl, br, cb, ro);
        ro = *(pk_gu32c*)(roff + (u + 192u) * 4u);
        pk_clade_entry<CL, CR>(B, u + 64u, (unsigned int)U, Pl, Pr, tabL, tabR, pi, ulik, flag);
    }
    if (nU & 1) pk_clade_entry<CL, CR>(A, u, (unsigned int)U, Pl, Pr, tabL, tabR, pi, ulik, flag);
    if (threadIdx.x == 0) ulik[U] = 1.0;
}
template <bool CL, bool CR>
__device__ __forceinline__ bool pk_rows_pat(int s1, const char* bl, const char* br, const char* rl, pk_pat_kargs* pa, const double (&Pl)[16],
                                            const double (&Pr)[16], const double (*tabL)[4], const double (*tabR)[4],
                                            const double (&pi)[4], double* ulik, pm_lp& col, unsigned int Z) {
    pm_lp_flag flag = pm_lp_flag_init();
    const char* pimg;
    pk_u4 n0, n1;
    if (pa->clade != nullptr) {
        const char* blk = pa->clade + (size_t)(Z * pa->cstride);
        pimg = blk + PK_CLADE_HDR_BYTES + pa->crep;
        if constexpr (CL || CR) pk_pat_request(n0, n1, pimg, 0);
        pk_clade_phase1<CL, CR>(blk, bl, br, rl, Pl, Pr, tabL, tabR, pi, ulik, flag);
        if constexpr (!(CL || CR)) pk_pat_request(n0, n1, pimg, 0);
    } else {
        pimg = pa->pimg;
        if constexpr (CL || CR) pk_pat_request(n0, n1, pimg, 0);
        pk_pat_phase1<CL, CR>(pa->U, bl, br, rl, pa->roff, Pl, Pr, tabL, tabR, pi, ulik, flag);
        if constexpr (!(CL || CR)) pk_pat_request(n0, n1, pimg, 0);
    }
    pk_wave_lds_fence();
    pk_pat_walk(s1, pimg, n0, n1, ulik, col, flag);
    return pm_lp_flag_set(flag);
}
template <bool CL, bool CR>
__device__ __forceinline__ pm_lp pk_rows_general_v(int s0, int s1, const char* bl, const char* br, const pk_cdbl* Pc, const pk_cdbl* pik,
                                                   double (*tabL)[4], double (*tabR)[4], double* lik25) {
    const double pi[4] = {pik[0], pik[1], pik[2], pik[3]};
    double Pl[16], Pr[16];
#pragma unroll
    for (int u = 0; u < 16; ++u) {
        Pl[u] = CL ? 0.0 : Pc[u];
        Pr[u] = CR ? 0.0 : Pc[16 + u];
    }
    pk_rowregs A;
    pm_lp col = pm_lp_init();
    if constexpr (CL || CR) {
        pk_cstream c;
        pk_cs_request<CL, CR>(c, bl, br, s0 >> 10);
        pk_rows_load_u<CL, CR>(A, bl, br, s0 + (int)(threadIdx.x & 63), s1);
        pk_rows_run_packed<CL, CR>(s0, s1, bl, br, A, c, Pl, Pr, tabL, tabR, lik25, pi, col);
    } else {
        pk_rows_load<CL, CR>(A, bl, br, s0 + (int)(threadIdx.x & 63), s1);
        pk_rows_run<CL, CR>(s0, s1, bl, br, A, Pl, Pr, tabL, tabR, lik25, pi, col);
    }
    return col;
}
__device__ __forceinline__ pm_lp pk_rows_general(unsigned int fl, int s0, int s1, const char* bl, const char* br, const double* Pu,
                                                 const double* pi4, double (*tabL)[4], double (*tabR)[4], double* lik25) {
    fl = (unsigned int)__builtin_amdgcn_readfirstlane((int)fl);
    s0 = __builtin_amdgcn_readfirstlane(s0);
    s1 = __builtin_amdgcn_readfirstlane(s1);
    bl = pk_uniform_ptr(bl);
    br = pk_uniform_ptr(br);
    const pk_cdbl* Pc = (const pk_cdbl*)pk_uniform_ptr(Pu);
    const pk_cdbl* pik = (const pk_cdbl*)pk_uniform_ptr(pi4);
    if ((fl & 3u) == 3u) return pk_rows_general_v<true, true>(s0, s1, bl, br, Pc, pik, tabL, tabR, lik25);
    if (fl & 1u) return pk_rows_general_v<true, false>(s0, s1, bl, br, Pc, pik, tabL, tabR, lik25);
    if (fl & 2u) return pk_rows_general_v<false, true>(s0, s1, bl, br, Pc, pik, tabL, tabR, lik25);
    return pk_rows_general_v<false, false>(s0, s1, bl, br, Pc, pik, tabL, tabR, lik25);
}
template <bool CL, bool CR>
__device__ __forceinline__ bool pk_rows_loop_pat(int s1, const char* bl, const char* br, const double* Pu, const pk_cdbl* Pc,
                                                 double (*tabL)[4], double (*tabR)[4], const pk_cdbl* pik, pm_lp& col, pk_pat_kargs* pa,
                                                 double* ulik, unsigned int Z) {
    static_assert(!(CL && CR), "an uncoded side");
    const double pi[4] = {pik[0], pik[1], pik[2], pik[3]};
    double Pl[16], Pr[16];
#pragma unroll
    for (int u = 0; u < 16; ++u) {
        Pl[u] = CL ? 0.0 : Pc[u];
        Pr[u] = CR ? 0.0 : Pc[16 + u];
    }
    const char* rl = nullptr;
    if constexpr (CL != CR) {
#pragma unroll
        for (int u = 0; u < 16; ++u) asm volatile("" : "+s"(CL ? Pr[u] : Pl[u]));
        rl = (CL ? bl : br) + pa->rep_delta;
        if constexpr (CL) pk_build_leaf_table(Pu, tabL, (int)(threadIdx.x & 63));
        else pk_build_leaf_table(Pu + 16, tabR, (int)(threadIdx.x & 63));
        pk_wave_lds_fence();
    }
    return __any(pk_rows_pat<CL, CR>(s1, bl, br, rl, pa, Pl, Pr, tabL, tabR, pi, ulik, col, Z));
}
template <bool CL, bool CR>
__device__ __forceinline__ bool pk_rows_loop_rec(int s0, int s1, const char* bl, const char* br, const double* Pu, const pk_cdbl* Pc,
                                                 double (*tabL)[4], double (*tabR)[4], double* lik25, const pk_cdbl* pik, pm_lp& col,
                                                 pk_pat_kargs* pa, double* ulik, unsigned int Z) {
    if constexpr (!(CL && CR)) {
        if (pa->U != 0) return pk_rows_loop_pat<CL, CR>(s1, bl, br, Pu, Pc, tabL, tabR, pik, col, pa, ulik, Z);
    }
    const int lane = threadIdx.x & 63;
    const double pi[4] = {pik[0], pik[1], pik[2], pik[3]};
    double Pl[16], Pr[16];
#pragma unroll
    for (int u = 0; u < 16; ++u) {
        Pl[u] = CL ? 0.0 : Pc[u];
        Pr[u] = CR ? 0.0 : Pc[16 + u];
    }
    if constexpr (CL != CR) {
#pragma unroll
        for (int u = 0; u < 16; ++u) asm volatile("" : "+s"(CL ? Pr[u] : Pl[u]));
    }
    pk_rowregs A;
    pk_cstream c;
    if constexpr (CL || CR) {
        pk_cs_request<CL, CR>(c, bl, br, s0 >> 10);
        pk_rows_load_u<CL, CR>(A, bl, br, s0 + lane, s1);
    } else {
        pk_rows_load<CL, CR>(A, bl, br, s0 + lane, s1);
    }
    bool redo = (s0 & 1023) != 0;
    if constexpr (CL && CR) {
        const bool special = pk_build_lik25_direct(Pu, pi, lik25, lane);
        if (lane == PK_PAD_CODE * 6) lik25[PK_PAD_CODE * 6] = 1.0;
        pk_wave_lds_fence();
        redo = redo || __any(special);
    } else if constexpr (CL) {
        pk_build_leaf_table(Pu, tabL, lane);
        pk_wave_lds_fence();
    } else if constexpr (CR) {
        pk_build_leaf_table(Pu + 16, tabR, lane);
        pk_wave_lds_fence();
    }
    if constexpr (CL || CR) {
        if (!redo) {
            bool flag;
            if constexpr (CL && CR) flag = pk_rows_fast_cc(s0, s1, bl, br, c, lik25, col);
            else flag = pk_rows_fast_mixed<CL, CR>(s0, s1, bl, br, A, c, Pl, Pr, tabL, tabR, pi, col);
            redo = __any(flag);
        }
        return redo;
    } else {
        pk_rows_run<CL, CR>(s0, s1, bl, br, A, Pl, Pr, tabL, tabR, lik25, pi, col);
        return false;
    }
}
struct pk_merge_kernarg { const unsigned long long* rec; const double* Pmat; int S, T, ntiles, n_xcd; double* tilev; pk_pi4 pi4; pk_pat_args pat; };
__global__ __launch_bounds__(64) __attribute__((amdgpu_waves_per_eu(7, 8), amdgpu_num_vgpr(32)))
void pk_rank_merge_nostore(const unsigned long long* __restrict__ rec, const double* __restrict__ Pmat, int S, int T, int ntiles,
                           int n_xcd, double* __restrict__ tilev, const pk_pi4 pi4, const pk_pat_args pat) {
    __shared__ __attribute__((aligned(16))) double tabL[PK_PAD_CODE + 1][4], tabR[PK_PAD_CODE + 1][4];
    __shared__ double lik25[PK_PAD_CODE * 6 + 1];
    extern __shared__ __attribute__((aligned(16))) double pk_ulik[];
    const int item = pk_launch_item((int)blockIdx.x, (int)gridDim.x, 1, 0, n_xcd < 0);
    if (item >= (n_xcd < 0 ? -n_xcd : n_xcd)) return;
    const int k = __builtin_amdgcn_readfirstlane(ntiles == 1 ? item : item / ntiles), tau = item - k * ntiles;
    const int s0 = __builtin_amdgcn_readfirstlane(tau * T), s1 = __builtin_amdgcn_readfirstlane(s0 + T < S ? s0 + T : S);
    const pk_cu64* rc = (const pk_cu64*)(rec + (size_t)k * PK_REC);
    const double* Pu = Pmat + (size_t)k * 32;
    const pk_cdbl* Pc = (const pk_cdbl*)Pu;
    PK_TOUCH4_DECL;
    PK_TOUCH4_256(Pu);
    unsigned int fl = (unsigned int)rc[REC_FLAGS];
    const char* bl = pk_uniform_ptr((const void*)rc[REC_BASE_L]);
    const char* br = pk_uniform_ptr((const void*)rc[REC_BASE_R]);
    PK_TOUCH4_END(fl);
    static_assert(offsetof(pk_merge_kernarg, pi4) == 40 && offsetof(pk_merge_kernarg, pat) == 72 && sizeof(pk_merge_kernarg) == 120,
                  "the kernel's argument segment");
    pk_pat_kargs* pa = (pk_pat_kargs*)((__attribute__((address_space(4))) const char*)__builtin_amdgcn_kernarg_segment_ptr() +
                                       offsetof(pk_merge_kernarg, pat));
    const pk_cdbl* pi = (const pk_cdbl*)((__attribute__((address_space(4))) const char*)__builtin_amdgcn_kernarg_segment_ptr() +
                                         offsetof(pk_merge_kernarg, pi4));
    pm_lp col = pm_lp_init();
    bool redo;
    if (fl & 1u) {
        if (fl & 2u) redo = pk_rows_loop_rec<true, true>(s0, s1, bl, br, Pu, Pc, tabL, tabR, lik25, pi, col, pa, pk_ulik, fl >> 2);
        else redo = pk_rows_loop_rec<true, false>(s0, s1, bl, br, Pu, Pc, tabL, tabR, lik25, pi, col, pa, pk_ulik, fl >> 2);
    } else {
        if (fl & 2u) redo = pk_rows_loop_rec<false, true>(s0, s1, bl, br, Pu, Pc, tabL, tabR, lik25, pi, col, pa, pk_ulik, fl >> 2);
        else redo = pk_rows_loop_rec<false, false>(s0, s1, bl, br, Pu, Pc, tabL, tabR, lik25, pi, col, pa, pk_ulik, fl >> 2);
    }
    if (redo) col = pk_rows_general(fl, s0, s1, bl, br, Pu, (const double*)pi, tabL, tabR, lik25);
    const double tot = pk_wave_tree_sum(pm_lp_finish(col));
    if (threadIdx.x == 0) {
        if (ntiles != 1) {
            tilev[(size_t)k * ntiles + tau] = tot;
        } else {
            const pk_cdbl* ax = (const pk_cdbl*)rc;
            const double fl2 = ax[AUX_SUM_REM] + tot;
            const double ll = ((fl2 + ax[AUX_FPRIOR]) + ax[AUX_LPRIOR]) + ax[AUX_RPRIOR];
            const double lw = (((ll - ax[AUX_LL_TILDE]) - ax[AUX_PAREN]) + ax[AUX_LOGV]) - ax[AUX_Q];
            *(pk_gd*)rc[REC_NODELL] = tot;
            *(pk_gd*)rc[REC_ROOTLL] = tot;
            *(pk_gd*)rc[REC_LL] = ll;
            *(pk_gd*)rc[REC_LOGW] = lw;
        }
    }
}

#define PK_MAX_SITE_TILE 4096
#define PK_STORE_STAGE_BYTES 8192
template <bool CL, bool CR, bool STORE>
__device__ __forceinline__ void pk_store_tile(int s0, int s1, int wv, int lane, const double* Lp, const double* Rp, const uint8_t* Lc,
                                              const uint8_t* Rc, double* out, const double (&Pl)[16], const double (&Pr)[16],
                                              const double (*tabL)[4], const double (*tabR)[4], const double (&pi)[4], double* likbuf,
                                              double* stage ) {
    const char* bl = pk_uniform_ptr(CL ? (const void*)Lc : (const void*)Lp);
    const char* br = pk_uniform_ptr(CR ? (const void*)Rc : (const void*)Rp);
    char* ob = const_cast<char*>(pk_uniform_ptr(out));
    pk_rowregs A, B;
    int u = s0 + 64 * wv;
    if (u >= s1) return;
    pk_rows_load<CL, CR>(A, bl, br, u + lane, s1);
    #pragma unroll 1
    for (; u < s1; u += 256) {
        pk_rows_load<CL, CR>(B, bl, br, u + 256 + lane, s1);
        double o[4];
        pk_rows_out<CL, CR>(A, Pl, Pr, tabL, tabR, o);
        const int s = u + lane;
        if (s < s1) likbuf[s - s0] = pk_site_lik(pi, o);
        if constexpr (STORE) {
            pk_d2* st = reinterpret_cast<pk_d2*>(stage);
// ... 570 lines not shown
```

### phylo_amd/csrc/phylo_math.h

```cpp
#pragma once
#include <stdint.h>

#if defined(__HIPCC__)
#define PM_HD __host__ __device__ __forceinline__
#else
#define PM_HD static inline
#endif

PM_HD uint64_t pm_bits(double x) { uint64_t u; __builtin_memcpy(&u, &x, 8); return u; }
PM_HD double pm_from_bits(uint64_t u) { double x; __builtin_memcpy(&x, &u, 8); return x; }
PM_HD double pm_fma(double a, double b, double c) { return __builtin_fma(a, b, c); }
PM_HD double pm_inf() { return pm_from_bits(0x7ff0000000000000ull); }
PM_HD double pm_nan() { return pm_from_bits(0x7ff8000000000000ull); }
PM_HD bool pm_isnan(double x) { return (pm_bits(x) & 0x7fffffffffffffffull) > 0x7ff0000000000000ull; }

PM_HD double pm_exp(double x) {
    const double o_threshold = 7.09782712893383973096e+02;
    const double u_threshold = -7.45133219101941108420e+02;
    const double ln2HI = 6.93147180369123816490e-01;
    const double ln2LO = 1.90821492927058770002e-10;
    const double invln2 = 1.44269504088896338700e+00;
    const double P1 = 1.66666666666666019037e-01;
    const double P2 = -2.77777777770155933842e-03;
    const double P3 = 6.61375632143793436117e-05;
// ... 18 lines not shown
        hi = x;
        lo = 0.0;
        r = x;
    }
    const double t = r * r;
    const double c = r - t * (P1 + t * (P2 + t * (P3 + t * (P4 + t * P5))));
    if (k == 0) return 1.0 - ((r * c) / (c - 2.0) - r);
    const double y = 1.0 - ((lo - (r * c) / (2.0 - c)) - hi);
    if (k >= -1021) return pm_from_bits(pm_bits(y) + ((uint64_t)(int64_t)k << 52));
    const double y2 = pm_from_bits(pm_bits(y) + ((uint64_t)(int64_t)(k + 1000) << 52));
    return y2 * 9.33263618503218878990e-302;
}

PM_HD double pm_exp_nonpos(double x) {
    const double u_threshold = -7.45133219101941108420e+02;
    const double ln2HI = 6.93147180369123816490e-01;
    const double ln2LO = 1.90821492927058770002e-10;
    const double invln2 = 1.44269504088896338700e+00;
    const double P1 = 1.66666666666666019037e-01;
    const double P2 = -2.77777777770155933842e-03;
    const double P3 = 6.61375632143793436117e-05;
    const double P4 = -1.65339022054652515390e-06;
    const double P5 = 4.13813679705723846039e-08;
    const double ax = -x;
    const double xc = x < -800.0 ? -800.0 : x;
    const int k = ax > 0.34657359027997264 ? (int)(invln2 * xc + -0.5) : 0;
    const double t = (double)k;
    const double hi = xc - t * ln2HI;
    const double lo = t * ln2LO;
    const double r = hi - lo;
    const double tt = r * r;
    const double c = r - tt * (P1 + tt * (P2 + tt * (P3 + tt * (P4 + tt * P5))));
    const double y = 1.0 - ((lo - (r * c) / (2.0 - c)) - hi);
    const double yn = pm_from_bits(pm_bits(y) + ((uint64_t)(int64_t)k << 52));
    const double ys = pm_from_bits(pm_bits(y) + ((uint64_t)(int64_t)(k + 1000) << 52)) * 9.33263618503218878990e-302;
    double res = k >= -1021 ? yn : ys;
    res = ax < 3.7252902984619141e-09 ? 1.0 + x : res;
    res = x < u_threshold ? 0.0 : res;
    return res;
}

PM_HD double pm_log(double x) {
    const double ln2_hi = 6.93147180369123816490e-01;
    const double ln2_lo = 1.90821492927058770002e-10;
    const double Lg1 = 6.666666666666735130e-01;
    const double Lg2 = 3.999999999940941908e-01;
    const double Lg3 = 2.857142874366239149e-01;
    const double Lg4 = 2.222219843214978396e-01;
    const double Lg5 = 1.818357216161805012e-01;
    const double Lg6 = 1.531383769920937332e-01;
    const double Lg7 = 1.479819860511658591e-01;
    uint64_t u = pm_bits(x);
    uint32_t hx = (uint32_t)(u >> 32);
    int k = 0;
    if (hx < 0x00100000u || (hx >> 31)) {
        if ((u << 1) == 0) return -pm_inf();
        if (hx >> 31) return pm_nan();
        k -= 54;
        x = x * 18014398509481984.0;
        u = pm_bits(x);
        hx = (uint32_t)(u >> 32);
    } else if (hx >= 0x7ff00000u) {
        return x;
    } else if (hx == 0x3ff00000u && (u << 32) == 0) {
        return 0.0;
    }
    hx += 0x3ff00000u - 0x3fe6a09eu;
    k += (int)(hx >> 20) - 0x3ff;
    hx = (hx & 0x000fffffu) + 0x3fe6a09eu;
    u = ((uint64_t)hx << 32) | (u & 0xffffffffull);
    x = pm_from_bits(u);
    const double f = x - 1.0;
    const double hfsq = 0.5 * f * f;
    const double s = f / (2.0 + f);
    const double z = s * s;
    const double w = z * z;
    const double t1 = w * (Lg2 + w * (Lg4 + w * Lg6));
    const double t2 = z * (Lg1 + w * (Lg3 + w * (Lg5 + w * Lg7)));
    const double R = t2 + t1;
    const double dk = (double)k;
    return s * (hfsq + R) + dk * ln2_lo - hfsq + f + dk * ln2_hi;
}

PM_HD int pm_site_tile(int S) { (void)S; return 2048; }

struct pm_lp { double p; int E; double extra; };

PM_HD pm_lp pm_lp_init() { pm_lp a = {1.0, 0, 0.0}; return a; }

PM_HD void pm_lp_mul(pm_lp& a, double x) {
    const uint64_t bx = pm_bits(x);
    const int ex = (int)((bx >> 52) & 0x7ff);
    if (bx - 0x0010000000000000ull >= 0x7fe0000000000000ull) {
        a.extra = a.extra + pm_log(x);
        return;
    }
    const double mx = pm_from_bits((bx & 0x000fffffffffffffull) | 0x3ff0000000000000ull);
    a.p = a.p * mx;
    const uint64_t bp = pm_bits(a.p);
    a.E += (ex - 1023) + ((int)((bp >> 52) & 0x7ff) - 1023);
    a.p = pm_from_bits((bp & 0x000fffffffffffffull) | 0x3ff0000000000000ull);
}

PM_HD void pm_lp_mul2(pm_lp& a, double x1, double x2) {
    const double q = (a.p * x1) * x2;
    const uint64_t bq = pm_bits(q);
    const uint32_t h1 = (uint32_t)(pm_bits(x1) >> 32), h2 = (uint32_t)(pm_bits(x2) >> 32), hq = (uint32_t)(bq >> 32);
    const bool ok = (h1 - 0x00100000u < 0x7fe00000u) & (h2 - 0x00100000u < 0x7fe00000u) & (hq - 0x00200000u < 0x7fd00000u);
    if (ok) {
        a.E += (int)(hq >> 20) - 1023;
        a.p = pm_from_bits((bq & 0x000fffffffffffffull) | 0x3ff0000000000000ull);
    } else {
        pm_lp_mul(a, x1);
        pm_lp_mul(a, x2);
    }
}

struct pm_lp_flag { uint32_t f, q; };
PM_HD pm_lp_flag pm_lp_flag_init() { pm_lp_flag g = {0xffffffffu, 0xffffffffu}; return g; }
PM_HD bool pm_lp_flag_set(const pm_lp_flag& g) { return (g.f < 0x80200000u) | (g.q < 0x80300000u); }
PM_HD uint32_t pm_lp_key(double x) { return (uint32_t)(pm_bits(x) >> 32) + 0x80100000u; }
PM_HD uint32_t pm_min_u32(uint32_t a, uint32_t b) { return a < b ? a : b; }
PM_HD bool pm_lp_special(double x) { return pm_bits(x) - 0x0010000000000000ull >= 0x7fe0000000000000ull; }
PM_HD void pm_lp_mul2_spec_q(pm_lp& a, double x1, double x2, pm_lp_flag& flag) {
    const double q = (a.p * x1) * x2;
    const uint64_t bq = pm_bits(q);
    flag.q = pm_min_u32(flag.q, pm_lp_key(q));
    a.E += (int)((uint32_t)(bq >> 32) >> 20) - 1023;
    a.p = pm_from_bits((bq & 0x000fffffffffffffull) | 0x3ff0000000000000ull);
}
PM_HD void pm_lp_mul2_spec(pm_lp& a, double x1, double x2, pm_lp_flag& flag) {
    flag.f = pm_min_u32(pm_min_u32(flag.f, pm_lp_key(x1)), pm_lp_key(x2));
    pm_lp_mul2_spec_q(a, x1, x2, flag);
}
PM_HD void pm_lp_mul_normal(pm_lp& a, double x) {
    const uint64_t bx = pm_bits(x);
    const int ex = (int)((bx >> 52) & 0x7ff);
    const double mx = pm_from_bits((bx & 0x000fffffffffffffull) | 0x3ff0000000000000ull);
    a.p = a.p * mx;
    const uint64_t bp = pm_bits(a.p);
    a.E += (ex - 1023) + ((int)((bp >> 52) & 0x7ff) - 1023);
    a.p = pm_from_bits((bp & 0x000fffffffffffffull) | 0x3ff0000000000000ull);
}
PM_HD void pm_lp_mul_spec(pm_lp& a, double x, pm_lp_flag& flag) {
    flag.f = pm_min_u32(flag.f, pm_lp_key(x));
    pm_lp_mul_normal(a, x);
}

PM_HD double pm_lp_finish(const pm_lp& a) {
    const double dE = (double)a.E;
    return ((pm_log(a.p) + dE * 1.90821492927058770002e-10) + dE * 6.93147180369123816490e-01) + a.extra;
}

struct pm_u32x4 { uint32_t x, y, z, w; };

PM_HD pm_u32x4 pm_philox4x32(uint32_t c0, uint32_t c1, uint32_t c2, uint32_t c3, uint64_t seed) {
    uint32_t k0 = (uint32_t)seed, k1 = (uint32_t)(seed >> 32);
#pragma unroll
    for (int i = 0; i < 10; ++i) {
        const uint64_t p0 = (uint64_t)0xD2511F53u * c0;
        const uint64_t p1 = (uint64_t)0xCD9E8D57u * c2;
        const uint32_t n0 = (uint32_t)(p1 >> 32) ^ c1 ^ k0;
        const uint32_t n1 = (uint32_t)p1;
        const uint32_t n2 = (uint32_t)(p0 >> 32) ^ c3 ^ k1;
        const uint32_t n3 = (uint32_t)p0;
        c0 = n0; c1 = n1; c2 = n2; c3 = n3;
        k0 += 0x9E3779B9u;
        k1 += 0xBB67AE85u;
    }
    pm_u32x4 r = {c0, c1, c2, c3};
    return r;
}

enum { PM_STREAM_PAIR = 0, PM_STREAM_BRANCH = 1, PM_STREAM_RESAMPLE = 2, PM_STREAM_TWIST = 3, PM_STREAM_BOOT = 4 };
#define PM_CDF_SCALE 17592186044416.0

PM_HD double pm_unit_oc(uint32_t lo, uint32_t hi) {
    const uint64_t b = ((uint64_t)hi << 32) | lo;
    return ((double)(b >> 11) + 1.0) * 1.1102230246251565404e-16;
}

PM_HD uint64_t pm_mulhi64(uint64_t a, uint64_t b) {
#if defined(__HIP_DEVICE_COMPILE__)
    return __umul64hi(a, b);
#else
    return (uint64_t)(((unsigned __int128)a * b) >> 64);
#endif
}

PM_HD uint64_t pm_weight_int(double logw, double m, bool all_bad) {
    if (all_bad) return 1ull;
    if (pm_isnan(logw)) return 0ull;
    return (uint64_t)(pm_exp(logw - m) * PM_CDF_SCALE);
}

PM_HD void pm_mm4(const double* a, const double* b, double* c) {
#pragma unroll
    for (int i = 0; i < 4; ++i)
#pragma unroll
        for (int j = 0; j < 4; ++j) {
            double acc = a[i * 4 + 0] * b[0 * 4 + j];
            acc = pm_fma(a[i * 4 + 1], b[1 * 4 + j], acc);
            acc = pm_fma(a[i * 4 + 2], b[2 * 4 + j], acc);
            acc = pm_fma(a[i * 4 + 3], b[3 * 4 + j], acc);
            c[i * 4 + j] = acc;
        }
}

PM_HD void pm_solve4(double* D, double* Nm) {
#pragma unroll
    for (int c = 0; c < 4; ++c) {
        int p = c;
        double best = D[c * 4 + c] < 0.0 ? -D[c * 4 + c] : D[c * 4 + c];
#pragma unroll
        for (int r = c + 1; r < 4; ++r) {
            const double v = D[r * 4 + c] < 0.0 ? -D[r * 4 + c] : D[r * 4 + c];
            if (v > best) { best = v; p = r; }
        }
#pragma unroll
        for (int r = c + 1; r < 4; ++r) {
            if (p == r) {
#pragma unroll
                for (int j = 0; j < 4; ++j) {
                    double t = D[c * 4 + j]; D[c * 4 + j] = D[r * 4 + j]; D[r * 4 + j] = t;
                    t = Nm[c * 4 + j]; Nm[c * 4 + j] = Nm[r * 4 + j]; Nm[r * 4 + j] = t;
                }
            }
        }
        const double piv = D[c * 4 + c];
#pragma unroll
// ... 129 lines not shown
```

### phylo_amd/csrc/phylo_persist.h

```cpp
#pragma once
#include "phylo_kernels.h"

#define PP_CHUNK 16
#define PP_CTR_STRIDE 16
#define PP_MAX_M 1024
#define PP_MAX_KG 8192
#define PP_SPIN_LIMIT (1u << 21)

struct pp_args {
    int N, S, K, Kg, G, R;
    int T;
    int Wg, m;
    uint64_t seed;
    const uint64_t* group_seeds;
    uint32_t flags;
    int jc;
    const double* Q; const double* lam_l; const double* lam_r; const double* pi; const double* ldf;
    const double* leaves; const uint8_t* leaf_codes; double* pool;
    int32_t* roots[2]; int32_t* cnt[2]; double* rootll[2];
    double* nodell; double* bl; double* br; double* Pmat; double* logw; double* ll;
    int32_t* child; int32_t* merges; int64_t* anc; unsigned int* mark;
    unsigned long long* rdraw;
    double* lse; int lse_stride;
    unsigned long long* ctr;
// ... 247 lines not shown
    uint64_t seed;
    uint32_t r_next;
};
template <int NT>
__device__ __forceinline__ void pp_scan_ancestors(const unsigned long long* cdf, int Kg, int g, const pp_anc_out& o, unsigned char* flag,
                                                  pp_scan_lds* sh) {
    constexpr int NW = NT / 64, ME = NT == 512 ? 8 : 16;
    const int tid = threadIdx.x, lane = tid & 63, wv = tid >> 6;
    for (int k = tid; k < Kg; k += NT) flag[k] = 0;
    __syncthreads();
    const uint64_t seed = o.group_seeds ? o.group_seeds[g] : o.seed;
    const unsigned long long total = cdf[Kg - 1];
    int32_t* anc = o.anc + (size_t)g * Kg;
    for (int base = 0; base < Kg; base += 4 * NT) {
        unsigned long long thr[4];
        int lo[4];
#pragma unroll
        for (int j = 0; j < 4; ++j) {
            const int k = base + tid + NT * j;
            const pm_u32x4 x = pm_philox4x32((uint32_t)(k < Kg ? k : Kg - 1), o.r_next, PM_STREAM_RESAMPLE, 0u, seed);
            thr[j] = pm_mulhi64(((uint64_t)x.y << 32) | x.x, total);
            lo[j] = 0;
        }
        for (int n = Kg; n > 1;) {
            const int half = n >> 1;
#pragma unroll
            for (int j = 0; j < 4; ++j) lo[j] = cdf[lo[j] + half - 1] > thr[j] ? lo[j] : lo[j] + half;
            n -= half;
        }
#pragma unroll
        for (int j = 0; j < 4; ++j) {
            const int k = base + tid + NT * j;
            if (k < Kg) { anc[k] = lo[j]; flag[lo[j]] = 1; }
        }
    }
    __syncthreads();
    const int E = (Kg + NT - 1) / NT;
    unsigned long long b[ME];
    int mine = 0;
#pragma unroll
    for (int j = 0; j < ME; ++j) {
        const int i = (wv * E + j) * 64 + lane;
        b[j] = __ballot(j < E && i < Kg && flag[i < Kg ? i : 0] != 0);
        mine += __popcll(b[j]);
    }
    if (lane == 0) sh->u[wv] = (unsigned long long)mine;
    __syncthreads();
    int off = 0, all = 0;
#pragma unroll
    for (int i = 0; i < NW; ++i) {
        const int u = (int)sh->u[i];
        if (i < wv) off += u;
        all += u;
    }
    int32_t* list = o.list + (size_t)g * Kg;
#pragma unroll
    for (int j = 0; j < ME; ++j) {
        if ((b[j] >> lane) & 1ull) list[off + __popcll(b[j] & ((1ull << lane) - 1ull))] = (wv * E + j) * 64 + lane;
        off += __popcll(b[j]);
    }
    if (tid == 0) o.cnt[g] = all;
}

template <int NT>
__global__ __launch_bounds__(NT) void pp_resample_scan(const double* logw, int Kg, uint64_t* __restrict__ cdf, double* lse_out, int lse_stride,
                                                       int logz_R) {
    extern __shared__ __attribute__((aligned(16))) char smem[];
    pp_scan_lds* sh = reinterpret_cast<pp_scan_lds*>(smem);
    unsigned long long* lcdf = reinterpret_cast<unsigned long long*>(smem + ((sizeof(pp_scan_lds) + 15) & ~(size_t)15));
    const int g = blockIdx.x;
    pp_scan<NT>(logw + (size_t)g * Kg, Kg, lcdf, lse_out ? lse_out + (size_t)g * lse_stride : (double*)nullptr, sh, cdf != nullptr);
    if (logz_R > 0 && lse_out && threadIdx.x == 0) {
        double* row = lse_out + (size_t)g * lse_stride - (logz_R - 1);
        double z = 0.0;
        for (int r = 0; r < logz_R; ++r) z = z + row[r];
        row[logz_R] = z;
    }
    if (!cdf) return;
    __syncthreads();
    unsigned long long* out = reinterpret_cast<unsigned long long*>(cdf) + (size_t)g * Kg;
    for (int k = threadIdx.x; k < Kg; k += NT) out[k] = lcdf[k];
}
template <int NT>
__global__ __launch_bounds__(NT) void pp_resample_scan_anc(const double* logw, int Kg, uint64_t* __restrict__ cdf, double* lse_out, int lse_stride,
                                                           const pp_anc_out ao) {
    extern __shared__ __attribute__((aligned(16))) char smem[];
    pp_scan_lds* sh = reinterpret_cast<pp_scan_lds*>(smem);
    unsigned long long* lcdf = reinterpret_cast<unsigned long long*>(smem + ((sizeof(pp_scan_lds) + 15) & ~(size_t)15));
    const int g = blockIdx.x;
    pp_scan<NT>(logw + (size_t)g * Kg, Kg, lcdf, lse_out ? lse_out + (size_t)g * lse_stride : (double*)nullptr, sh, true);
    pp_scan_ancestors<NT>(lcdf, Kg, g, ao, reinterpret_cast<unsigned char*>(lcdf + Kg), sh);
    unsigned long long* out = reinterpret_cast<unsigned long long*>(cdf) + (size_t)g * Kg;
    for (int k = threadIdx.x; k < Kg; k += NT) out[k] = lcdf[k];
}
#define PP_SCAN_TILE 2048
struct pp_scan_multi_args {
    const double* logw;
    int Kg, B;
    double* gmax;
    unsigned long long* bsum;
    unsigned long long* wbits;
    unsigned long long* cdf;
    double* lse_out;
    int lse_stride, logz_R;
    int lse_only;
};
__device__ __forceinline__ double pp_scan_multi_group_max(const pp_scan_multi_args& a, int g) {
    double m = pp_gld(a.gmax + (size_t)g * a.B);
    for (int b = 1; b < a.B; ++b) {
        const double o = pp_gld(a.gmax + (size_t)g * a.B + b);
        m = o > m ? o : m;
    }
    return m;
}
__global__ __launch_bounds__(512) void pp_scan_multi_max(const pp_scan_multi_args a) {
    __shared__ double sh[8];
    const int b = blockIdx.x, g = blockIdx.y, tid = threadIdx.x, lane = tid & 63, wv = tid >> 6;
    const double* logw = a.logw + (size_t)g * a.Kg;
    double m = -pm_inf();
#pragma unroll
    for (int j = 0; j < 4; ++j) {
        const int k = b * PP_SCAN_TILE + tid + 512 * j;
        const double v = pp_gld(logw + (k < a.Kg ? k : a.Kg - 1));
        if (k < a.Kg && !pm_isnan(v) && v > m) m = v;
    }
    m = pp_wave_max(m);
    if (lane == 0) sh[wv] = m;
    __syncthreads();
    if (tid == 0) {
        m = sh[0];
#pragma unroll
        for (int i = 1; i < 8; ++i) m = sh[i] > m ? sh[i] : m;
        a.gmax[(size_t)g * a.B + b] = m;
    }
}
__global__ __launch_bounds__(512) void pp_scan_multi_exp(const pp_scan_multi_args a) {
    __shared__ unsigned long long sh[8];
    const int b = blockIdx.x, g = blockIdx.y, tid = threadIdx.x, lane = tid & 63, wv = tid >> 6;
    const double* logw = a.logw + (size_t)g * a.Kg;
    const double m = pp_scan_multi_group_max(a, g);
    const bool all_bad = !(m > -pm_inf()) || m == pm_inf();
    double v[4], w[4];
#pragma unroll
    for (int j = 0; j < 4; ++j) {
        const int k = b * PP_SCAN_TILE + tid + 512 * j;
        v[j] = pp_gld(logw + (k < a.Kg ? k : a.Kg - 1));
    }
#pragma unroll
    for (int j = 0; j < 4; ++j) {
        const bool nan = pm_isnan(v[j]);
        const double e = pm_exp_nonpos(nan ? 0.0 : v[j] - m);
        w[j] = all_bad ? 1.0 : (nan ? 0.0 : e);
    }
    unsigned long long local = 0;
#pragma unroll
    for (int j = 0; j < 4; ++j) {
        const int k = b * PP_SCAN_TILE + tid + 512 * j;
        if (k < a.Kg) {
            a.wbits[(size_t)g * a.Kg + k] = pm_bits(w[j]);
            local += all_bad ? 1ull : (unsigned long long)(w[j] * PM_CDF_SCALE);
        }
    }
    const unsigned long long incl = pp_wave_incl_scan_u64(local, lane);
    if (lane == 63) sh[wv] = incl;
    __syncthreads();
    if (tid == 0) {
        unsigned long long t = 0;
#pragma unroll
        for (int i = 0; i < 8; ++i) t += sh[i];
        a.bsum[(size_t)g * a.B + b] = t;
    }
}
__global__ __launch_bounds__(512) void pp_scan_multi_cdf(const pp_scan_multi_args a) {
    __shared__ pp_scan_lds sh;
    const int b = blockIdx.x, g = blockIdx.y, tid = threadIdx.x, lane = tid & 63, wv = tid >> 6;
    const unsigned long long* wb = a.wbits + (size_t)g * a.Kg;
// ... 533 lines not shown
```

Measured before the change: 763.4 billion particle-site-likelihoods/s.

## Drop cdf writes in ancestor scan, tame-path lp multiply, DPP lane reductions, log table

```diff
diff --git a/phylo_amd/csrc/phylo_hip.hip b/phylo_amd/csrc/phylo_hip.hip
--- a/phylo_amd/csrc/phylo_hip.hip
+++ b/phylo_amd/csrc/phylo_hip.hip
@@ -133,6 +133,7 @@
     int jc = 0;
     std::vector<double> h_lam_l, h_lam_r, h_ldf;
     double *d_Q = nullptr, *d_pi = nullptr, *d_lam_l = nullptr, *d_lam_r = nullptr, *d_ldf = nullptr;
+    double* d_logv = nullptr;
     double* d_leaves = nullptr;
     uint8_t* d_leaf_codes = nullptr;
     uint8_t* d_leaf_packed = nullptr;
@@ -643,9 +644,9 @@
 int launch_scan(phylo_ctx* c, const double* logw, int Kg, int G, uint64_t* cdf, double* lse, int lse_stride, int logz_R = 0,
                 const pp_anc_out* anc = nullptr) {
     const pp_anc_out ao = anc ? *anc : pp_anc_out{};
-    const sweep_scan_form form = sweep_scan_form_of(Kg, c->env.scan_multi_min, cdf || lse, k_sweep_limits);
-    if (ao.anc && (!cdf || logz_R > 0 || (form != SCAN_LDS_512 && form != SCAN_LDS_1024)))
-        return fail(c, PHYLO_ESTATE, "launch_scan: the resampling outcome needs a cdf and a scan that holds it in LDS (Kg = %d)", Kg);
+    const sweep_scan_form form = sweep_scan_form_of(Kg, c->env.scan_multi_min, cdf || lse || ao.anc, k_sweep_limits);
+    if (ao.anc && (cdf || logz_R > 0 || (form != SCAN_LDS_512 && form != SCAN_LDS_1024)))
+        return fail(c, PHYLO_ESTATE, "launch_scan: the resampling outcome needs a scan that holds the cdf in LDS, and writes none (Kg = %d)", Kg);
     if (form == SCAN_MULTI) {
         pp_scan_multi_args a{};
         a.logw = logw; a.Kg = Kg; a.B = (Kg + PP_SCAN_TILE - 1) / PP_SCAN_TILE;
@@ -663,7 +664,7 @@
         return launch_check(c, "pp_scan_multi_cdf");
     }
     if (form == SCAN_LDS_512) {
-        if (ao.anc) hipLaunchKernelGGL(pp_resample_scan_anc<512>, dim3(G), dim3(512), pp_resample_scan_lds(Kg, true), c->stream, logw, Kg, cdf, lse, lse_stride, ao);
+        if (ao.anc) hipLaunchKernelGGL(pp_resample_scan_anc<512>, dim3(G), dim3(512), pp_resample_scan_lds(Kg, true), c->stream, logw, Kg, lse, lse_stride, ao);
         else hipLaunchKernelGGL(pp_resample_scan<512>, dim3(G), dim3(512), pp_resample_scan_lds(Kg), c->stream, logw, Kg, cdf, lse, lse_stride, logz_R);
         return launch_check(c, "pp_resample_scan");
     }
@@ -681,7 +682,7 @@
                                               (int)pp_resample_scan_lds(PP_SCAN_KERNEL_MAX_KG, true)));
                 raised_anc = true;
             }
-            hipLaunchKernelGGL(pp_resample_scan_anc<1024>, dim3(G), dim3(1024), lds, c->stream, logw, Kg, cdf, lse, lse_stride, ao);
+            hipLaunchKernelGGL(pp_resample_scan_anc<1024>, dim3(G), dim3(1024), lds, c->stream, logw, Kg, lse, lse_stride, ao);
             return launch_check(c, "pp_resample_scan_anc");
         }
         hipLaunchKernelGGL(pp_resample_scan<1024>, dim3(G), dim3(1024), lds, c->stream, logw, Kg, cdf, lse, lse_stride, logz_R);
@@ -773,14 +774,16 @@
         c->d_pi = c->d_Q + 16;
         c->d_lam_l = c->d_Q + 20;
         c->d_lam_r = c->d_Q + 20 + N;
-        if ((rc = dalloc(c, &c->d_ldf, (size_t)N + 1)) != PHYLO_OK) break;
+        if ((rc = dalloc(c, &c->d_ldf, (size_t)N + 1 + pm_log_table_len(N))) != PHYLO_OK) break;
+        c->d_logv = c->d_ldf + N + 1;
         if ((rc = dalloc(c, &c->d_leaves, (size_t)N * S * 4)) != PHYLO_OK) break;
         if ((rc = dalloc(c, &c->d_leaf_codes, pk_leaf_image_bytes(N, S))) != PHYLO_OK) break;
         c->d_leaf_packed = c->d_leaf_codes + pk_packed_offset(N, S);
         c->d_pat = c->d_leaf_codes + pk_pat_offset(N, S);
-        c->h_ldf.resize((size_t)N + 1);
+        c->h_ldf.resize((size_t)N + 1 + pm_log_table_len(N));
         for (int cnt = 0; cnt <= N; ++cnt) c->h_ldf[cnt] = host_log_double_factorial(2 * (cnt > 2 ? cnt : 2) - 3);
-        if (hipMemcpy(c->d_ldf, c->h_ldf.data(), ((size_t)N + 1) * 8, hipMemcpyHostToDevice) != hipSuccess) { rc = fail(c, PHYLO_EHIP, "ldf upload failed"); break; }
+        pm_fill_log_table(c->h_ldf.data() + N + 1, pm_log_table_len(N));
+        if (hipMemcpy(c->d_ldf, c->h_ldf.data(), c->h_ldf.size() * 8, hipMemcpyHostToDevice) != hipSuccess) { rc = fail(c, PHYLO_EHIP, "ldf upload failed"); break; }
     } while (0);
     if (rc != PHYLO_OK) {
         g_last_error = c->err;
@@ -2640,6 +2643,9 @@
     b.ll_prev = r > 0 ? c->d_ll + (size_t)(r - 1) * K : nullptr;
     b.nodell = c->d_nodell;
     b.ldf = c->d_ldf; b.ldf_n = N;
+    b.logv = c->d_logv;
+    b.q_pair = 1.0 / ((double)((b.n - 1) * b.n) / 2.0);
+    b.logq_pair = pm_log(b.q_pair);
     b.bl = c->d_bl; b.br = c->d_br;
     b.lam_l = c->h_lam_l[r]; b.lam_r = c->h_lam_r[r];
     b.loglam_l = pm_log(b.lam_l); b.loglam_r = pm_log(b.lam_r);
@@ -2865,7 +2871,7 @@
         ao.anc = c->d_anc_next; ao.list = c->d_adopt_list; ao.cnt = c->d_adopt_cnt;
         ao.group_seeds = p.G > 1 ? c->d_group_seeds : nullptr; ao.seed = c->run.seed; ao.r_next = (uint32_t)(r + 1);
     }
-    return launch_scan(c, (const double*)(c->d_logw + (size_t)r * c->K), p.Kg, p.G, last ? (uint64_t*)nullptr : c->d_cdf[(r & 1) ^ 1],
+    return launch_scan(c, (const double*)(c->d_logw + (size_t)r * c->K), p.Kg, p.G, (last || ao.anc) ? (uint64_t*)nullptr : c->d_cdf[(r & 1) ^ 1],
                        c->d_lse + r, p.lse_stride, (last && p.fold_logz) ? p.R : 0, ao.anc ? &ao : nullptr);
 }
 
@@ -4002,9 +4008,8 @@
     if (!logw || !seeds || !anc || !list || !cnt || Kg < 1 || G < 1 || G > PK_MAX_GROUPS)
         return fail(c, PHYLO_EINVAL, "phylo_debug_scan_ancestors: bad arguments");
     const size_t K = (size_t)Kg * G;
-    void *dw, *dcdf, *dout, *dseed;
+    void *dw, *dout, *dseed;
     CHK(scratch_get(c, 0, K * 8, &dw));
-    CHK(scratch_get(c, 1, K * 8, &dcdf));
     CHK(scratch_get(c, 2, (2 * K + (size_t)G) * 4, &dout));
     CHK(scratch_get(c, 3, (size_t)G * 8, &dseed));
     HIPCHK(c, hipMemcpyAsync(dw, logw, K * 8, hipMemcpyHostToDevice, c->stream));
@@ -4013,7 +4018,7 @@
     pp_anc_out ao{};
     ao.anc = (int32_t*)dout; ao.list = ao.anc + K; ao.cnt = ao.list + K;
     ao.group_seeds = (const uint64_t*)dseed; ao.r_next = r_next;
-    CHK(launch_scan(c, (const double*)dw, Kg, G, (uint64_t*)dcdf, (double*)nullptr, 0, 0, &ao));
+    CHK(launch_scan(c, (const double*)dw, Kg, G, (uint64_t*)nullptr, (double*)nullptr, 0, 0, &ao));
     HIPCHK(c, hipMemcpyAsync(anc, ao.anc, K * 4, hipMemcpyDeviceToHost, c->stream));
     HIPCHK(c, hipMemcpyAsync(list, ao.list, K * 4, hipMemcpyDeviceToHost, c->stream));
     HIPCHK(c, hipMemcpyAsync(cnt, ao.cnt, (size_t)G * 4, hipMemcpyDeviceToHost, c->stream));
diff --git a/phylo_amd/csrc/phylo_kernels.h b/phylo_amd/csrc/phylo_kernels.h
--- a/phylo_amd/csrc/phylo_kernels.h
+++ b/phylo_amd/csrc/phylo_kernels.h
@@ -550,6 +550,7 @@
     const double* ll_prev;
     double* nodell;
     const double* ldf; int ldf_n;
+    const double* logv; double q_pair, logq_pair;
     const double* bl; const double* br;
     double lam_l, lam_r, loglam_l, loglam_r, ll_tilde0;
     const double* leaves;
@@ -687,6 +688,33 @@
     return lo;
 }
 
+template <int LP, int OFF>
+__device__ __forceinline__ int pk_lanes_partner(int v) {
+    if constexpr (LP > 16) return __shfl_xor(v, OFF, 64);
+    else if constexpr (OFF == 1) return __builtin_amdgcn_update_dpp(0, v, 0xB1 , 0xf, 0xf, true);
+    else if constexpr (OFF == 2) return __builtin_amdgcn_update_dpp(0, v, 0x4E , 0xf, 0xf, true);
+    else if constexpr (OFF == 4) return __builtin_amdgcn_update_dpp(0, v, 0x141 , 0xf, 0xf, true);
+    else return __builtin_amdgcn_update_dpp(0, v, 0x140 , 0xf, 0xf, true);
+}
+template <int LP, int OFF>
+__device__ __forceinline__ unsigned long long pk_lanes_partner64(unsigned long long v) {
+    const unsigned int lo = (unsigned int)pk_lanes_partner<LP, OFF>((int)(unsigned int)v);
+    const unsigned int hi = (unsigned int)pk_lanes_partner<LP, OFF>((int)(unsigned int)(v >> 32));
+    return ((unsigned long long)hi << 32) | lo;
+}
+template <int LP, int OFF = 1>
+__device__ __forceinline__ unsigned long long pk_lanes_max64(unsigned long long v) {
+    if constexpr (OFF < LP) {
+        const unsigned long long o = pk_lanes_partner64<LP, OFF>(v);
+        return pk_lanes_max64<LP, OFF * 2>(o > v ? o : v);
+    } else return v;
+}
+template <int LP, int OFF = 1>
+__device__ __forceinline__ int pk_lanes_sum(int v) {
+    if constexpr (OFF < LP) return pk_lanes_sum<LP, OFF * 2>(v + pk_lanes_partner<LP, OFF>(v));
+    else return v;
+}
+
 template <int LP, bool KEY_LOOP, bool ANC_IN = false, bool BITS = false>
 __device__ __forceinline__ void pk_book_packed(const pk_rank_args& a, int kg, bool local, const pk_book_lds& L, int sl, int lane) {
     const int n = a.n, N = a.N, k = kg - a.k0;
@@ -756,11 +784,7 @@
             const unsigned long long c = ((unsigned long long)L.key[i] << 32) | (0xffffffffu - (uint32_t)i);
             best = c > best ? c : best;
         }
-#pragma unroll
-        for (int off = 1; off < LP; off <<= 1) {
-            const unsigned long long o = __shfl_xor(best, off, 64);
-            best = o > best ? o : best;
-        }
+        best = pk_lanes_max64<LP>(best);
         const int il = (int)(0xffffffffu - (uint32_t)best);
         best = 0ull;
         #pragma unroll 1
@@ -768,11 +792,7 @@
             const unsigned long long c = ((unsigned long long)L.key[i] << 32) | (0xffffffffu - (uint32_t)i);
             if (i != il) best = c > best ? c : best;
         }
-#pragma unroll
-        for (int off = 1; off < LP; off <<= 1) {
-            const unsigned long long o = __shfl_xor(best, off, 64);
-            best = o > best ? o : best;
-        }
+        best = pk_lanes_max64<LP>(best);
         const int ir = (int)(0xffffffffu - (uint32_t)best);
         int32_t* rn = a.roots_new + (size_t)kg * N;
         int32_t* cn = a.cnt_new + (size_t)kg * N;
@@ -836,10 +856,9 @@
             const int c = L.ord_cnt[p];
             vminus += c - (c == 1 ? 1 : 0);
         }
-#pragma unroll
-        for (int off = 1; off < LP; off <<= 1) vminus += __shfl_xor(vminus, off, 64);
-        const double q = 1.0 / ((double)((n - 1) * n) / 2.0);
-        const double lg = pm_log(sl == 0 ? (double)vminus : q);
+        vminus = pk_lanes_sum<LP>(vminus);
+        const double q = a.q_pair;
+        const double lg = sl == 0 ? a.logv[vminus] : a.logq_pair;
         if (sl == 0) {
             const double b_l = L.hbl[a.r], b_r = L.hbr[a.r];
             L.aux[AUX_SUM_REM] = acc;
@@ -1646,15 +1665,14 @@
         for (int j = 0; j < 4; ++j) o[j] = tl[j] * tr[j];
         const double x = pk_site_lik(pi, o);
         lik25[t] = x;
-        special = pm_lp_special(x);
+        special = !pm_lp_tame(x);
     }
     return special;
 }
 __device__ __forceinline__ unsigned int pk_cw_byte(const unsigned int (&w)[4], int j) { return (w[j >> 2] >> (8 * (j & 3))) & 0xffu; }
-__device__ __forceinline__ bool pk_rows_fast_cc(int s0, int s1, const char* bl, const char* br, pk_cstream& c, const double* lik25,
+__device__ __forceinline__ void pk_rows_fast_cc(int s0, int s1, const char* bl, const char* br, pk_cstream& c, const double* lik25,
                                                 pm_lp& col) {
     const char* lb = (const char*)lik25;
-    pm_lp_flag flag = pm_lp_flag_init();
     int n = __builtin_amdgcn_readfirstlane((s1 - s0 + 63) >> 6), Jc = __builtin_amdgcn_readfirstlane(s0 >> 10);
     #pragma unroll 1
     for (;;) {
@@ -1669,12 +1687,11 @@
             }
             const double xa = *(const double*)(lb + pk_cw_byte(w, j));
             const double xb = *(const double*)(lb + pk_cw_byte(w, j + 1));
-            pm_lp_mul2_spec_q(col, xa, xb, flag);
+            pm_lp_mul2_tame(col, xa, xb);
         }
         if (n <= 16) break;
         n -= 16; ++Jc;
     }
-    return pm_lp_flag_set(flag);
 }
 template <bool CL, bool CR>
 __device__ __forceinline__ void pk_rows_pair_spec(pk_rowregs& A, pk_rowregs& B, unsigned int ca, unsigned int cb, int s, int s1,
@@ -1735,18 +1752,18 @@
 template <bool CL, bool CR>
 __device__ __forceinline__ void pk_pat_entry(pk_rowregs& X, unsigned int code, unsigned int u, unsigned int U, const double (&Pl)[16],
                                              const double (&Pr)[16], const double (*tabL)[4], const double (*tabR)[4],
-                                             const double (&pi)[4], double* ulik, pm_lp_flag& flag) {
+                                             const double (&pi)[4], double* ulik, uint32_t& worst) {
     if constexpr (CL) X.cl = code;
     if constexpr (CR) X.cr = code;
     double x = pk_rows_lik<CL, CR>(X, Pl, Pr, tabL, tabR, nullptr, pi);
     x = u < U ? x : 1.0;
-    flag.f = pm_min_u32(flag.f, pm_lp_key(x));
+    worst = pm_max_u32(worst, pm_lp_tame_key(x));
     ulik[u] = x;
 }
 template <bool CL, bool CR>
 __device__ __forceinline__ void pk_pat_phase1(int U, const char* bl, const char* br, const char* rl, const char* roff,
                                               const double (&Pl)[16], const double (&Pr)[16], const double (*tabL)[4],
-                                              const double (*tabR)[4], const double (&pi)[4], double* ulik, pm_lp_flag& flag) {
+                                              const double (*tabR)[4], const double (&pi)[4], double* ulik, uint32_t& worst) {
     static_assert(!(CL && CR), "an uncoded side");
     const int nU = __builtin_amdgcn_readfirstlane((U + 63) >> 6);
     unsigned int u = threadIdx.x & 63u;
@@ -1764,13 +1781,13 @@
         pk_pat_rows<CL, CR>(B, bl, br, ro);
         ro = *(pk_gu32c*)(roff + (u + 128u) * 4u);
         const unsigned int cw = (unsigned int)lo;
-        pk_pat_entry<CL, CR>(A, cw & 0xffu, u, (unsigned int)U, Pl, Pr, tabL, tabR, pi, ulik, flag);
+        pk_pat_entry<CL, CR>(A, cw & 0xffu, u, (unsigned int)U, Pl, Pr, tabL, tabR, pi, ulik, worst);
         pk_pat_rows<CL, CR>(A, bl, br, ro);
         ro = *(pk_gu32c*)(roff + (u + 192u) * 4u);
-        pk_pat_entry<CL, CR>(B, (cw >> 8) & 0xffu, u + 64u, (unsigned int)U, Pl, Pr, tabL, tabR, pi, ulik, flag);
+        pk_pat_entry<CL, CR>(B, (cw >> 8) & 0xffu, u + 64u, (unsigned int)U, Pl, Pr, tabL, tabR, pi, ulik, worst);
         lo >>= 16;
     }
-    if (nU & 1) pk_pat_entry<CL, CR>(A, (unsigned int)lo & 0xffu, u, (unsigned int)U, Pl, Pr, tabL, tabR, pi, ulik, flag);
+    if (nU & 1) pk_pat_entry<CL, CR>(A, (unsigned int)lo & 0xffu, u, (unsigned int)U, Pl, Pr, tabL, tabR, pi, ulik, worst);
     if (threadIdx.x == 0) ulik[U] = 1.0;
 }
 __device__ __forceinline__ void pk_pat_request(pk_u4& n0, pk_u4& n1, const char* pimg, int Jc) {
@@ -1778,7 +1795,7 @@
     n0 = *(pk_gu4c*)(pimg + o);
     n1 = *(pk_gu4c*)(pimg + o + (unsigned int)PK_PAT_HALF_BYTES);
 }
-__device__ __forceinline__ void pk_pat_walk(int s1, const char* pimg, pk_u4 n0, pk_u4 n1, const double* ulik, pm_lp& col, pm_lp_flag& flag) {
+__device__ __forceinline__ void pk_pat_walk(int s1, const char* pimg, pk_u4 n0, pk_u4 n1, const double* ulik, pm_lp& col) {
     const char* ub = (const char*)ulik;
     int n = __builtin_amdgcn_readfirstlane((s1 + 63) >> 6), Jc = 0;
     #pragma unroll 1
@@ -1793,7 +1810,7 @@
             }
             const double xa = *(const double*)(ub + (w[j >> 1] & 0xffffu));
             const double xb = *(const double*)(ub + (w[j >> 1] >> 16));
-            pm_lp_mul2_spec_q(col, xa, xb, flag);
+            pm_lp_mul2_tame(col, xa, xb);
         }
         if (n <= 16) break;
         n -= 16; ++Jc;
@@ -1814,16 +1831,16 @@
 template <bool CL, bool CR>
 __device__ __forceinline__ void pk_clade_entry(const pk_rowregs& X, unsigned int u, unsigned int U, const double (&Pl)[16],
                                                const double (&Pr)[16], const double (*tabL)[4], const double (*tabR)[4],
-                                               const double (&pi)[4], double* ulik, pm_lp_flag& flag) {
+                                               const double (&pi)[4], double* ulik, uint32_t& worst) {
     double x = pk_rows_lik<CL, CR>(X, Pl, Pr, tabL, tabR, nullptr, pi);
     x = u < U ? x : 1.0;
-    flag.f = pm_min_u32(flag.f, pm_lp_key(x));
+    worst = pm_max_u32(worst, pm_lp_tame_key(x));
     ulik[u] = x;
 }
 template <bool CL, bool CR>
 __device__ __forceinline__ void pk_clade_phase1(const char* blk, const char* bl, const char* br, const char* cb, const double (&Pl)[16],
                                                 const double (&Pr)[16], const double (*tabL)[4], const double (*tabR)[4],
-                                                const double (&pi)[4], double* ulik, pm_lp_flag& flag) {
+                                                const double (&pi)[4], double* ulik, uint32_t& worst) {
     static_assert(!(CL && CR), "an uncoded side");
     const char* roff = blk + PK_CLADE_HDR_BYTES;
     unsigned int u = threadIdx.x & 63u;
@@ -1837,36 +1854,36 @@
     for (int t = 0; t < (nU >> 1); ++t, u += 128u) {
         pk_clade_rows<CL, CR>(B, bl, br, cb, ro);
         ro = *(pk_gu32c*)(roff + (u + 128u) * 4u);
-        pk_clade_entry<CL, CR>(A, u, (unsigned int)U, Pl, Pr, tabL, tabR, pi, ulik, flag);
+        pk_clade_entry<CL, CR>(A, u, (unsigned int)U, Pl, Pr, tabL, tabR, pi, ulik, worst);
         pk_clade_rows<CL, CR>(A, bl, br, cb, ro);
         ro = *(pk_gu32c*)(roff + (u + 192u) * 4u);
-        pk_clade_entry<CL, CR>(B, u + 64u, (unsigned int)U, Pl, Pr, tabL, tabR, pi, ulik, flag);
-    }
-    if (nU & 1) pk_clade_entry<CL, CR>(A, u, (unsigned int)U, Pl, Pr, tabL, tabR, pi, ulik, flag);
+        pk_clade_entry<CL, CR>(B, u + 64u, (unsigned int)U, Pl, Pr, tabL, tabR, pi, ulik, worst);
+    }
+    if (nU & 1) pk_clade_entry<CL, CR>(A, u, (unsigned int)U, Pl, Pr, tabL, tabR, pi, ulik, worst);
     if (threadIdx.x == 0) ulik[U] = 1.0;
 }
 template <bool CL, bool CR>
 __device__ __forceinline__ bool pk_rows_pat(int s1, const char* bl, const char* br, const char* rl, pk_pat_kargs* pa, const double (&Pl)[16],
                                             const double (&Pr)[16], const double (*tabL)[4], const double (*tabR)[4],
                                             const double (&pi)[4], double* ulik, pm_lp& col, unsigned int Z) {
-    pm_lp_flag flag = pm_lp_flag_init();
+    uint32_t worst = 0;
     const char* pimg;
     pk_u4 n0, n1;
     if (pa->clade != nullptr) {
         const char* blk = pa->clade + (size_t)(Z * pa->cstride);
         pimg = blk + PK_CLADE_HDR_BYTES + pa->crep;
         if constexpr (CL || CR) pk_pat_request(n0, n1, pimg, 0);
-        pk_clade_phase1<CL, CR>(blk, bl, br, rl, Pl, Pr, tabL, tabR, pi, ulik, flag);
+        pk_clade_phase1<CL, CR>(blk, bl, br, rl, Pl, Pr, tabL, tabR, pi, ulik, worst);
         if constexpr (!(CL || CR)) pk_pat_request(n0, n1, pimg, 0);
     } else {
         pimg = pa->pimg;
         if constexpr (CL || CR) pk_pat_request(n0, n1, pimg, 0);
-        pk_pat_phase1<CL, CR>(pa->U, bl, br, rl, pa->roff, Pl, Pr, tabL, tabR, pi, ulik, flag);
+        pk_pat_phase1<CL, CR>(pa->U, bl, br, rl, pa->roff, Pl, Pr, tabL, tabR, pi, ulik, worst);
         if constexpr (!(CL || CR)) pk_pat_request(n0, n1, pimg, 0);
     }
     pk_wave_lds_fence();
-    pk_pat_walk(s1, pimg, n0, n1, ulik, col, flag);
-    return pm_lp_flag_set(flag);
+    pk_pat_walk(s1, pimg, n0, n1, ulik, col);
+    return !pm_lp_tame_keys(worst);
 }
 template <bool CL, bool CR>
 __device__ __forceinline__ pm_lp pk_rows_general_v(int s0, int s1, const char* bl, const char* br, const pk_cdbl* Pc, const pk_cdbl* pik,
@@ -1970,10 +1987,8 @@
     }
     if constexpr (CL || CR) {
         if (!redo) {
-            bool flag;
-            if constexpr (CL && CR) flag = pk_rows_fast_cc(s0, s1, bl, br, c, lik25, col);
-            else flag = pk_rows_fast_mixed<CL, CR>(s0, s1, bl, br, A, c, Pl, Pr, tabL, tabR, pi, col);
-            redo = __any(flag);
+            if constexpr (CL && CR) pk_rows_fast_cc(s0, s1, bl, br, c, lik25, col);
+            else redo = __any(pk_rows_fast_mixed<CL, CR>(s0, s1, bl, br, A, c, Pl, Pr, tabL, tabR, pi, col));
         }
         return redo;
     } else {
diff --git a/phylo_amd/csrc/phylo_math.h b/phylo_amd/csrc/phylo_math.h
--- a/phylo_amd/csrc/phylo_math.h
+++ b/phylo_amd/csrc/phylo_math.h
@@ -124,6 +124,11 @@
     return s * (hfsq + R) + dk * ln2_lo - hfsq + f + dk * ln2_hi;
 }
 
+PM_HD int pm_log_table_len(int N) { return 2 * N + 2; }
+PM_HD void pm_fill_log_table(double* t, int len) {
+    for (int v = 0; v < len; ++v) t[v] = pm_log((double)v);
+}
+
 PM_HD int pm_site_tile(int S) { (void)S; return 2048; }
 
 struct pm_lp { double p; int E; double extra; };
@@ -188,6 +193,26 @@
     flag.f = pm_min_u32(flag.f, pm_lp_key(x));
     pm_lp_mul_normal(a, x);
 }
+PM_HD uint32_t pm_lp_tame_key(double x) { return (uint32_t)(pm_bits(x) >> 32) - 0x20100000u; }
+PM_HD uint32_t pm_max_u32(uint32_t a, uint32_t b) { return a > b ? a : b; }
+PM_HD bool pm_lp_tame_keys(uint32_t worst) { return worst < 0x5fe00000u - 0x20100000u; }
+PM_HD bool pm_lp_tame(double x) { return pm_lp_tame_keys(pm_lp_tame_key(x)); }
+PM_HD uint32_t pm_lp_mant_hi(uint32_t h) {
+#if defined(__HIP_DEVICE_COMPILE__)
+    uint32_t r;
+    asm("v_bfi_b32 %0, %1, %2, %3" : "=v"(r) : "s"(0x000fffffu), "v"(h), "v"(0x3ff00000u));
+    return r;
+#else
+    return (h & 0x000fffffu) | 0x3ff00000u;
+#endif
+}
+PM_HD void pm_lp_mul2_tame(pm_lp& a, double x1, double x2) {
+    const double q = (a.p * x1) * x2;
+    const uint64_t bq = pm_bits(q);
+    const uint32_t hq = (uint32_t)(bq >> 32);
+    a.E += (int)(hq >> 20) - 1023;
+    a.p = pm_from_bits(((uint64_t)pm_lp_mant_hi(hq) << 32) | (bq & 0xffffffffull));
+}
 
 PM_HD double pm_lp_finish(const pm_lp& a) {
     const double dE = (double)a.E;
diff --git a/phylo_amd/csrc/phylo_persist.h b/phylo_amd/csrc/phylo_persist.h
--- a/phylo_amd/csrc/phylo_persist.h
+++ b/phylo_amd/csrc/phylo_persist.h
@@ -353,16 +353,13 @@
     for (int k = threadIdx.x; k < Kg; k += NT) out[k] = lcdf[k];
 }
 template <int NT>
-__global__ __launch_bounds__(NT) void pp_resample_scan_anc(const double* logw, int Kg, uint64_t* __restrict__ cdf, double* lse_out, int lse_stride,
-                                                           const pp_anc_out ao) {
+__global__ __launch_bounds__(NT) void pp_resample_scan_anc(const double* logw, int Kg, double* lse_out, int lse_stride, const pp_anc_out ao) {
     extern __shared__ __attribute__((aligned(16))) char smem[];
     pp_scan_lds* sh = reinterpret_cast<pp_scan_lds*>(smem);
     unsigned long long* lcdf = reinterpret_cast<unsigned long long*>(smem + ((sizeof(pp_scan_lds) + 15) & ~(size_t)15));
     const int g = blockIdx.x;
     pp_scan<NT>(logw + (size_t)g * Kg, Kg, lcdf, lse_out ? lse_out + (size_t)g * lse_stride : (double*)nullptr, sh, true);
     pp_scan_ancestors<NT>(lcdf, Kg, g, ao, reinterpret_cast<unsigned char*>(lcdf + Kg), sh);
-    unsigned long long* out = reinterpret_cast<unsigned long long*>(cdf) + (size_t)g * Kg;
-    for (int k = threadIdx.x; k < Kg; k += NT) out[k] = lcdf[k];
 }
 #define PP_SCAN_TILE 2048
 struct pp_scan_multi_args {
```

Measured after the change: 780.2 billion particle-site-likelihoods/s (median of 5 runs). +2.2%, better.
